# swarth100/dynfu

Measured on AMD Instinct MI355X. Metric: frames/sec (warp-solve + TSDF fuse), 512^3 vol / 2k nodes / VGA depth, higher is better.
Workload: dtype f32; 1 GPU; C2: 512^3 TSDF, 640x480 depth, 2048 nodes, k=4, 262144 vertices, 5 GN x PCG<=256 (tol 1e-6), reference-parity energy (energy.t), lambda=200; parallelism=replicas x1 (one sequence per GPU, no collective), ranks_seen=1, repeats=5

## Files before the change

### dynfu_amd/csrc/capi.cpp

```cpp
#include <hip/hip_runtime.h>

#include <cmath>
#include <cstdarg>
#include <cstdio>
#include <cstring>
#include <map>
#include <mutex>
#include <new>
#include <utility>
#include <vector>

#include "../../include/dynfu_amd.h"
#include "kernels.hpp"
#include "dev_switch.hpp"
#include "solve.hpp"
#include "solve6.hpp"

namespace {

thread_local char g_err[512] = "";

int fail(int code, const char* fmt, ...) {
    va_list ap;
    va_start(ap, fmt);
    vsnprintf(g_err, sizeof(g_err), fmt, ap);
    va_end(ap);
    return code;
}

int hip_fail(hipError_t e, const char* what) {
    return fail(e == hipErrorNoDevice ? DFA_ERR_NO_GPU : DFA_ERR_HIP, "%s: %s", what, hipGetErrorString(e));
}

#define REQUIRE(cond, msg) \
    if (!(cond)) return fail(DFA_ERR_INVALID, "%s: %s", __func__, msg)
#define HIP_TRY(expr)                                  \
    do {                                               \
        hipError_t e_ = (expr);                        \
        if (e_ != hipSuccess) return hip_fail(e_, #expr); \
    } while (0)

inline hipStream_t S(dfa_stream_t s) { return (hipStream_t)s; }

bool volume_args_ok(const void* vol, int X, int Y, int Z) { return vol && X > 0 && Y > 0 && Z > 0; }

template <class T>
T& stream_scratch(hipStream_t s) {
    static std::mutex mu;
    static std::map<std::pair<int, hipStream_t>, T> table;
    int dev = 0;
    (void)hipGetDevice(&dev);
    std::lock_guard<std::mutex> lock(mu);
    return table[std::make_pair(dev, s)];
}

struct GridScratch {
    dfa::KnnGridView v{};
    int cap_nodes = 0;
    void release() {
        (void)hipFree(v.desc), (void)hipFree(v.cell_count), (void)hipFree(v.cell_start);
        (void)hipFree(v.node_cell), (void)hipFree(v.sorted);
        v         = dfa::KnnGridView{};
        cap_nodes = 0;
    }
    hipError_t reserve(int D_needed) {
        if (D_needed <= cap_nodes) return hipSuccess;
        const int D = D_needed + D_needed / 4 + 64;
        release();
        hipError_t e;
        if ((e = hipMalloc((void**)&v.desc, sizeof(dfa::KnnGridDesc))) != hipSuccess) return e;
        if ((e = hipMalloc((void**)&v.cell_count, sizeof(int32_t) * dfa::KNN_GRID_MAX_CELLS)) != hipSuccess) return e;
        if ((e = hipMalloc((void**)&v.cell_start, sizeof(int32_t) * (dfa::KNN_GRID_MAX_CELLS + 1))) != hipSuccess)
            return e;
        if ((e = hipMalloc((void**)&v.node_cell, sizeof(int32_t) * (size_t)D)) != hipSuccess) return e;
        if ((e = hipMalloc((void**)&v.sorted, sizeof(float4) * (size_t)D)) != hipSuccess) return e;
        cap_nodes = D;
        return hipSuccess;
    }
};

struct PointGridScratch {
    dfa::PointGridView v{};
    int cap_points = 0;
    void release() {
        (void)hipFree(v.g.desc), (void)hipFree(v.g.cell_count), (void)hipFree(v.g.cell_start);
        (void)hipFree(v.g.node_cell), (void)hipFree(v.g.sorted), (void)hipFree(v.chunk_sums);
        (void)hipFree(v.bbox_partials);
        v          = dfa::PointGridView{};
        cap_points = 0;
    }
    hipError_t reserve(int n_needed) {
        if (n_needed <= cap_points) return hipSuccess;
        const int n = n_needed + n_needed / 4 + 1024;
        release();
        hipError_t e;
        const size_t cells = dfa::PGRID_MAX_CELLS;
        if ((e = hipMalloc((void**)&v.g.desc, sizeof(dfa::KnnGridDesc))) != hipSuccess) return e;
        if ((e = hipMalloc((void**)&v.g.cell_count, sizeof(int32_t) * cells)) != hipSuccess) return e;
        if ((e = hipMalloc((void**)&v.g.cell_start, sizeof(int32_t) * (cells + 1))) != hipSuccess) return e;
        if ((e = hipMalloc((void**)&v.g.node_cell, sizeof(int32_t) * (size_t)n)) != hipSuccess) return e;
        if ((e = hipMalloc((void**)&v.g.sorted, sizeof(float4) * (size_t)n)) != hipSuccess) return e;
        if ((e = hipMalloc((void**)&v.chunk_sums, sizeof(int32_t) * (cells / dfa::PGRID_CHUNK))) != hipSuccess) return e;
        if ((e = hipMalloc((void**)&v.bbox_partials, sizeof(float) * 6 * dfa::PGRID_BBOX_BLOCKS)) != hipSuccess) return e;
        cap_points = n;
        return hipSuccess;
    }
};

struct McScratch {
    int32_t* seg_off    = nullptr;
    int32_t* chunk_sums = nullptr;
    long cap_segs       = 0;
    hipError_t reserve(long nsegs) {
        if (nsegs <= cap_segs) return hipSuccess;
        (void)hipFree(seg_off), (void)hipFree(chunk_sums);
        seg_off = chunk_sums = nullptr, cap_segs = 0;
        hipError_t e;
        if ((e = hipMalloc((void**)&seg_off, sizeof(int32_t) * (size_t)(nsegs + 1))) != hipSuccess) return e;
        if ((e = hipMalloc((void**)&chunk_sums, sizeof(int32_t) * (size_t)dfa::mc_scan_chunks(nsegs))) != hipSuccess)
            return e;
        cap_segs = nsegs;
        return hipSuccess;
    }
};
struct McIndexedScratch {
    McScratch vert;
    int32_t* idx_off = nullptr;
    long cap_segs    = 0;
    hipError_t reserve(long nsegs) {
        hipError_t e = vert.reserve(nsegs);
        if (e != hipSuccess || nsegs <= cap_segs) return e;
        (void)hipFree(idx_off);
        idx_off = nullptr, cap_segs = 0;
        if ((e = hipMalloc((void**)&idx_off, sizeof(int32_t) * (size_t)(nsegs + 1))) != hipSuccess) return e;
        cap_segs = nsegs;
        return hipSuccess;
    }
};

bool want_grid(int D, long n_query) { return D >= 64 && ((long)D * n_query >= (1L << 22) || D >= 1024); }

}

struct dfa_solver {
    int max_D, max_N, k;
    size_t max_R;
    int ell_cap;
    dfa::SolveView v;
    dfa::SolveState* state;
    double* cost_partials;
    unsigned int* ticket;
    std::vector<void*> blocks;
    GridScratch grid;
    bool has_problem;
    bool timing;
    std::vector<hipEvent_t> events;
    std::vector<int> ev_pcg, ev_asm;
    size_t ev_used;
    int timed_solves = 0;
    dfa::MbGraphCache mb_graphs;
    dfa::TeamPcg team;
    bool deterministic = false;
    bool just_reset = false;
    long long* iters_total = nullptr;
    dfa_overlap_fn overlap_fn = nullptr;
    void* overlap_user        = nullptr;
    int* host_flag = nullptr;
};

struct dfa_solver6 {
    int max_D, max_N, k;
    dfa::Solve6View v;
    dfa::Solve6State* state;
    float* raw_w;
    int32_t* raw_reg;
    const float* node_dq;
    std::vector<void*> blocks;
    GridScratch grid;
    bool has_problem;
    std::map<int, hipGraphExec_t> pcg_graphs;
    int last_launches = 0;
    static constexpr int S6_RING = 4;
    int* mirror = nullptr;
    hipEvent_t done_ev[S6_RING] = {};
    int slot_gn[S6_RING] = {};
    unsigned long long solve_seq = 0, folded = 0;
    int pred[dfa::S6_HIST] = {};
    struct BudgetKey { int D, N, num_iter, gn_iter, linear_iter; float tol, tol_first, tol_decay, tol_adapt, gn_tol; } budget_key = {};
    bool graph_disabled = false;
    hipStream_t capture_stream = nullptr;
    bool timing = false;
    std::vector<hipEvent_t> events;
    size_t ev_used = 0;
    int pcg_key_D = -1;
};

namespace {
template <class T>
int plan6_alloc(dfa_solver6* s, T** out, size_t count) {
    void* p      = nullptr;
    hipError_t e = hipMalloc(&p, sizeof(T) * (count ? count : 1));
    if (e != hipSuccess) return hip_fail(e, "hipMalloc (solver6 plan)");
    s->blocks.push_back(p);
    *out = (T*)p;
    return DFA_OK;
}
}

namespace {
int timing_begin(dfa_solver* s, hipStream_t st) {
    if (s->ev_used + 2 > s->events.size()) {
        for (int i = 0; i < 2; ++i) {
            hipEvent_t e;
            if (hipEventCreate(&e) != hipSuccess) return -1;
            s->events.push_back(e);
        }
    }
    const int idx = (int)s->ev_used;
    s->ev_used += 2;
    (void)hipEventRecord(s->events[idx], st);
    return idx;
}
void timing_end(dfa_solver* s, int idx, hipStream_t st) {
    if (idx >= 0) (void)hipEventRecord(s->events[idx + 1], st);
}

template <class T>
int plan_alloc(dfa_solver* s, T** out, size_t count) {
    void* p       = nullptr;
    hipError_t e  = hipMalloc(&p, sizeof(T) * (count ? count : 1));
    if (e != hipSuccess) return hip_fail(e, "hipMalloc (solver plan)");
    s->blocks.push_back(p);
    *out = (T*)p;
    return DFA_OK;
}
}

extern "C" {

const char* dfa_last_error(void) { return g_err; }

const char* dfa_version(void) { return "dynfu_amd 0.1 (gfx950, HIP)"; }

int dfa_abi_version(void) { return DFA_ABI_VERSION; }

size_t dfa_abi_struct_size(int id) {
    switch (id) {
        case DFA_STRUCT_SOLVE_PARAMS: return sizeof(dfa_solve_params);
        case DFA_STRUCT_SOLVE_STATS: return sizeof(dfa_solve_stats);
        case DFA_STRUCT_SOLVE_TIMING: return sizeof(dfa_solve_timing);
        case DFA_STRUCT_SOLVE6_PARAMS: return sizeof(dfa_solve6_params);
        case DFA_STRUCT_SOLVE6_STATS: return sizeof(dfa_solve6_stats);
        case DFA_STRUCT_SOLVE6_TIMING: return sizeof(dfa_solve6_timing);
        default: return 0;
    }
}


int dfa_compute_dists(const uint16_t* depth, int depth_step, uint16_t* dists, int dists_step, int cols, int rows,
                      float fx, float fy, float cx, float cy, dfa_stream_t stream) {
    REQUIRE(depth && dists, "null image");
    REQUIRE(cols > 0 && rows > 0, "empty image");
    REQUIRE(depth_step >= cols * 2 && dists_step >= cols * 2, "row step smaller than a row");
    REQUIRE(fx != 0.f && fy != 0.f, "zero focal length");
    HIP_TRY(dfa::launch_compute_dists(depth, depth_step, dists, dists_step, cols, rows, fx, fy, cx, cy, S(stream)));
    return DFA_OK;
}

int dfa_tsdf_clear(uint32_t* volume, int X, int Y, int Z, dfa_stream_t stream) {
    REQUIRE(volume_args_ok(volume, X, Y, Z), "bad volume");
    HIP_TRY(dfa::launch_tsdf_clear(volume, X, Y, Z, S(stream)));
    return DFA_OK;
}

size_t dfa_tsdf_occupancy_bytes(int X, int Y, int Z) {
    return X > 0 && Y > 0 && Z > 0 ? dfa::occ_dims(X, Y, Z).bytes() : 0;
}

int dfa_tsdf_clear_occ(uint32_t* volume, int X, int Y, int Z, uint8_t* occupancy, dfa_stream_t stream) {
    REQUIRE(volume_args_ok(volume, X, Y, Z), "bad volume");
    REQUIRE(occupancy, "null occupancy map");
    HIP_TRY(dfa::launch_tsdf_clear(volume, X, Y, Z, S(stream)));
    HIP_TRY(hipMemsetAsync(occupancy, 0, dfa::occ_dims(X, Y, Z).bytes(), S(stream)));
    return DFA_OK;
}

static int integrate_common(bool fused, const uint16_t* dists, int dists_step, int cols, int rows, uint32_t* volume,
                            int X, int Y, int Z, const float voxel_size[3], float trunc_dist, int max_weight,
                            const float vol2cam[12], float fx, float fy, float cx, float cy, uint8_t* occupancy,
                            dfa_stream_t stream, bool occupancy_known = false) {
    REQUIRE(volume_args_ok(volume, X, Y, Z), "bad volume");
    REQUIRE(dists && cols > 0 && rows > 0 && dists_step >= cols * 2, "bad dists image");
    REQUIRE(voxel_size && vol2cam, "null parameter block");
    REQUIRE(trunc_dist > 0.f, "trunc_dist must be positive");
    REQUIRE(max_weight >= 0 && max_weight <= 65535, "max_weight must fit the 16-bit weight");
    HIP_TRY(dfa::launch_tsdf_integrate(fused, dists, dists_step, cols, rows, volume, X, Y, Z, voxel_size, trunc_dist,
                                       max_weight, vol2cam, fx, fy, cx, cy, occupancy, occupancy_known, S(stream)));
    return DFA_OK;
}

int dfa_tsdf_integrate_occ(const uint16_t* dists, int dists_step, int cols, int rows, uint32_t* volume, int X, int Y, int Z,
                           const float voxel_size[3], float trunc_dist, int max_weight, const float vol2cam[12], float fx,
                           float fy, float cx, float cy, uint8_t* occupancy, dfa_stream_t stream) {
    REQUIRE(occupancy, "null occupancy map");
    return integrate_common(false, dists, dists_step, cols, rows, volume, X, Y, Z, voxel_size, trunc_dist, max_weight, vol2cam,
                            fx, fy, cx, cy, occupancy, stream);
}

int dfa_tsdf_clear_integrate_occ(const uint16_t* dists, int dists_step, int cols, int rows, uint32_t* volume, int X, int Y,
                                 int Z, const float voxel_size[3], float trunc_dist, int max_weight,
                                 const float vol2cam[12], float fx, float fy, float cx, float cy, uint8_t* occupancy,
                                 dfa_stream_t stream) {
    REQUIRE(occupancy, "null occupancy map");
    return integrate_common(true, dists, dists_step, cols, rows, volume, X, Y, Z, voxel_size, trunc_dist, max_weight, vol2cam,
                            fx, fy, cx, cy, occupancy, stream);
}
// ... 507 lines not shown
        grid = &gs.v;
    }
    HIP_TRY(dfa::launch_correspond(canon_vertices, canon_normals, n_canon, live_vertices, n_live, out_vertices,
                                   out_normals, out_index, grid, S(stream)));
    return DFA_OK;
}

int dfa_correspond_projective(const float* vertices, const float* normals, int n, const float* vmap, int vmap_step,
                              const float* nmap, int nmap_step, int cols, int rows, float fx, float fy, float cx, float cy,
                              float dist_thresh, float min_cosine, float* out_vertices, float* out_normals,
                              int32_t* out_pixel, dfa_stream_t stream) {
    REQUIRE(n >= 0 && (n == 0 || vertices), "bad vertices");
    REQUIRE(vmap && cols > 0 && rows > 0 && vmap_step >= 16 * cols, "bad vertex map");
    REQUIRE(!nmap || nmap_step >= 16 * cols, "bad normal map pitch");
    REQUIRE(!out_normals || nmap, "normals requested without a normal map");
    REQUIRE(fx > 0.f && fy > 0.f && dist_thresh >= 0.f, "bad intrinsics / threshold");
    REQUIRE(((uintptr_t)vmap & 15) == 0 && (vmap_step & 15) == 0 && ((uintptr_t)nmap & 15) == 0 && (!nmap || (nmap_step & 15) == 0),
            "maps must be 16-byte aligned float4 images");
    HIP_TRY(dfa::launch_correspond_projective(vertices, normals, n, vmap, vmap_step, nmap, nmap_step, cols, rows, fx, fy, cx,
                                              cy, dist_thresh, min_cosine, out_vertices, out_normals, out_pixel,
                                              S(stream)));
    return DFA_OK;
}


int dfa_solver_create(int max_D, int max_N, int k, dfa_solver** out) {
    REQUIRE(out, "null out");
    *out = nullptr;
    REQUIRE(max_D > 0 && max_N >= 0, "bad sizes");
    REQUIRE(k >= 1 && k <= DFA_MAX_KNN, "k out of range 1..16");
    REQUIRE(max_D <= dfa::solve_pcg_max_nodes(), "more nodes than a plan supports (32768)");
    int ndev = 0;
    if (hipGetDeviceCount(&ndev) != hipSuccess || ndev == 0) return fail(DFA_ERR_NO_GPU, "no HIP device");
    dfa_solver* s = new (std::nothrow) dfa_solver();
    REQUIRE(s, "out of host memory");
    s->max_D = max_D, s->max_N = max_N, s->k = k;
    s->max_R       = (size_t)max_N + (size_t)max_D * k;
    s->ell_cap     = 256;
    s->has_problem = false;
    s->timing      = false;
    {
        const char* e    = getenv("DFA_ASSEMBLE_DETERMINISTIC");
        s->deterministic = e && atoi(e) != 0;
    }
    s->ev_used     = 0;
    std::memset(&s->v, 0, sizeof(s->v));
    const size_t R = s->max_R, D = (size_t)max_D;
    int rc = DFA_OK;
#define A(field, count) \
    if (rc == DFA_OK) rc = plan_alloc(s, &s->v.field, (count))
    A(ridx, R * k);
    A(rw, R * k);
    A(rtau, R);
    A(rb, R * 3);
    A(re, R * (size_t)dfa::solve_rec_words(k));
    A(reg_idx, D * k);
    A(blk_hist, D * (dfa::SOLVE_TG_BLOCKS + 1));
    A(node_ptr, D + 1);
    A(node_list, R * k);
    A(ell, D * s->ell_cap);
    A(ell_cnt, D);
    A(diag, D);
    A(g, D * 3);
    A(g_base, D * 3);
    A(t_base, D * 3);
    A(pk_perm, D);
    A(pk_perm2, D);
    A(pk_vals, D * s->ell_cap);
    A(pk_cols, D * s->ell_cap);
    A(mb_x, D);
    A(mb_r, D);
    A(mb_p, D);
    A(mb_s, D);
    A(mb_w, D);
    A(mb_u[0], D);
    A(mb_u[1], D);
    A(mb_m[0], D);
    A(mb_m[1], D);
    A(mb_t[0], D);
    A(mb_t[1], D);
    A(mb_gpart[0], (size_t)dfa::solve_mb_blocks(max_D));
    A(mb_gpart[1], (size_t)dfa::solve_mb_blocks(max_D));
    A(mb_dpart[0], (size_t)dfa::solve_mb_blocks(max_D));
    A(mb_dpart[1], (size_t)dfa::solve_mb_blocks(max_D));
    A(t, D * 3);
    A(huber, D);
    A(node_dq_out, D * 8);
#undef A
    if (rc == DFA_OK) {
        hipError_t e = s->grid.reserve(max_D);
        if (e != hipSuccess) rc = hip_fail(e, "hipMalloc (node grid)");
    }
    if (rc == DFA_OK && dfa::solve_team_pcg_fits(max_D) && (max_D > 2048 || dfa::kDevAB)) {
        s->v.team_stride = (max_D + 3) & ~3;
        rc = plan_alloc(s, &s->v.team_ctl, 1);
        const size_t areas = (size_t)3 * dfa::solve_team_pcg_rounds();
        if (rc == DFA_OK) rc = plan_alloc(s, &s->v.team_mt, areas * s->v.team_stride);
        if (rc == DFA_OK) rc = plan_alloc(s, &s->v.team_words, dfa::solve_team_pcg_words());
        if (rc == DFA_OK && (hipMemset(s->v.team_ctl, 0, sizeof(dfa::TeamCtl)) != hipSuccess ||
                             hipMemset(s->v.team_words, 0, sizeof(unsigned long long) * dfa::solve_team_pcg_words()) != hipSuccess ||
                             hipMemset(s->v.team_mt, 0, sizeof(float2) * areas * (size_t)s->v.team_stride) != hipSuccess))
            rc = fail(DFA_ERR_HIP, "hipMemset (team PCG)");
        if (rc == DFA_OK && hipHostMalloc((void**)&s->team.host_abort, sizeof(int), hipHostMallocDefault) == hipSuccess) {
            *s->team.host_abort = 0;
            s->team.ctl = s->v.team_ctl;
            if (const char* e0 = dfa::dev_env("DFA_MB_TEAM_EPOCH")) s->team.epoch = (unsigned)std::strtoul(e0, nullptr, 0);
        }
    }
    if (rc == DFA_OK) rc = plan_alloc(s, &s->state, 1);
    if (rc == DFA_OK) rc = plan_alloc(s, &s->iters_total, 1);
    if (rc == DFA_OK && hipMemset(s->iters_total, 0, sizeof(long long)) != hipSuccess) rc = DFA_ERR_HIP;
    if (rc == DFA_OK && hipHostMalloc((void**)&s->host_flag, 4 * sizeof(int), hipHostMallocDefault) != hipSuccess) s->host_flag = nullptr;
    if (rc == DFA_OK) rc = plan_alloc(s, &s->cost_partials, std::max<size_t>((R + 255) / 256 + 1, 1024) + 1024);
    if (rc == DFA_OK) rc = plan_alloc(s, &s->ticket, 64);
    if (rc == DFA_OK && hipMemset(s->ticket, 0, 64 * sizeof(unsigned int)) != hipSuccess)
        rc = fail(DFA_ERR_HIP, "hipMemset (ticket)");
    if (rc != DFA_OK) {
        dfa_solver_destroy(s);
        return rc;
    }
    *out = s;
    return DFA_OK;
}

void dfa_solver_destroy(dfa_solver* s) {
    if (!s) return;
    for (void* p : s->blocks) (void)hipFree(p);
    s->grid.release();
    for (hipEvent_t e : s->events) (void)hipEventDestroy(e);
    if (s->host_flag) (void)hipHostFree(s->host_flag);
    if (s->team.host_abort) (void)hipHostFree(s->team.host_abort);
    s->mb_graphs.release();
    delete s;
}

int dfa_solver_set_problem(dfa_solver* s, const float* node_pos, const float* node_dq, const float* node_w, int D,
                           const float* canon_vertices, const float* canon_normals, const float* live_vertices,
                           const float* live_normals, int N, dfa_stream_t stream) {
    (void)canon_normals;
    (void)live_normals;
    REQUIRE(s, "null plan");
    REQUIRE(node_pos && node_dq && node_w && D > 0, "no nodes");
    REQUIRE(N >= 0 && (N == 0 || (canon_vertices && live_vertices)), "bad vertex arrays");
    if (D > s->max_D || N > s->max_N)
        return fail(DFA_ERR_CAPACITY, "dfa_solver_set_problem: D=%d N=%d exceed the plan (max_D=%d max_N=%d)", D, N,
                    s->max_D, s->max_N);
    dfa::SolveView& v = s->v;
    v.N = N, v.D = D, v.k = s->k, v.Dpad = (D + 3) & ~3, v.ell_cap = s->ell_cap;
    v.deterministic = s->deterministic ? 1 : 0;
    v.node_pos = node_pos, v.node_dq = node_dq, v.node_w = node_w;
    v.canon = canon_vertices, v.live = live_vertices;
    hipStream_t st = S(stream);
    const dfa::KnnGridView* grid = nullptr;
    if (want_grid(D, (long)N + D)) {
        HIP_TRY(dfa::knn_grid_build(s->grid.v, node_pos, D, st));
        grid = &s->grid.v;
    }
    if (N > 0) HIP_TRY(dfa::launch_knn(node_pos, node_w, D, canon_vertices, N, s->k, v.ridx, v.rw, grid, st));
    HIP_TRY(dfa::launch_knn(node_pos, node_w, D, node_pos, D, s->k, v.reg_idx, nullptr, grid, st));
    HIP_TRY(dfa::solve_build_graph(v, s->state, s->ticket, 64, st));
    s->has_problem = true;
    s->just_reset  = true;
    return DFA_OK;
}

int dfa_solver_set_deterministic(dfa_solver* s, int on) {
    REQUIRE(s, "null plan");
    s->deterministic = on != 0;
    return DFA_OK;
}

int dfa_solver_solve(dfa_solver* s, const dfa_solve_params* p, dfa_stream_t stream) {
    REQUIRE(s && p, "null plan / params");
    REQUIRE(s->has_problem, "set_problem has not been called");
    REQUIRE(p->num_iter >= 0 && p->nonlinear_iter >= 0 && p->linear_iter >= 0, "negative iteration count");
    REQUIRE(p->tukey_offset > 0.f && p->psi_data > 0.f, "tukey_offset / psi_data must be positive");
    REQUIRE(p->lambda >= 0.f && std::isfinite(p->lambda), "lambda must be non-negative and finite");
    const dfa::SolveView& v = s->v;
    hipStream_t st          = S(stream);
    if (!s->just_reset) HIP_TRY(dfa::solve_reset(v, s->state, s->ticket, 64, st));
    s->just_reset = false;
    const double w_reg    = std::sqrt((double)p->lambda / ((double)v.D * (double)v.k));
    const float w_reg_f   = (float)w_reg;
    const float w_reg_sq  = w_reg_f * w_reg_f;
    if (s->timing) s->timed_solves += 1;
    if (s->host_flag) s->host_flag[0] = s->host_flag[1] = 0;
    s->mb_graphs.call = 0;
    int not_launched = 0;
    int gn_launched = 0;
    bool huber_done = false;
    const bool big_budget = (long)p->num_iter * p->nonlinear_iter > 8;
    const bool pcg_async  = dfa::solve_pcg_is_async(v, &s->team, p->linear_iter);
    const bool no_regradient = dfa::dev_env("DFA_NO_REGRADIENT") != nullptr;
    for (int outer = 0; outer < p->num_iter; ++outer) {
        if (s->host_flag && s->host_flag[1] == 2) s->host_flag[1] = 0;
        int gn_in_outer = 0;
        for (int gn = 0; gn < p->nonlinear_iter; ++gn) {
            if (big_budget && gn_in_outer >= 4 && gn_in_outer % 4 == 0 && s->host_flag && !s->host_flag[1] && pcg_async) {
                HIP_TRY(hipMemcpyAsync(&s->host_flag[1], &s->state->converged, sizeof(int), hipMemcpyDeviceToHost, st));
                HIP_TRY(hipStreamSynchronize(st));
            }
            if (s->host_flag && s->host_flag[1]) {
                ++not_launched;
                continue;
            }
            ++gn_in_outer;
            if (gn > 0 && p->gn_tol == 0.f && p->lambda > 0.f && !no_regradient) {
                int evg = s->timing ? timing_begin(s, st) : -1;
                HIP_TRY(dfa::solve_regradient(v, s->state, st));
                timing_end(s, evg, st);
                if (evg >= 0) s->ev_asm.push_back(evg);
                if (s->overlap_fn) s->overlap_fn(s->overlap_user, stream, gn_launched);
                ++gn_launched;
                int evr = s->timing ? timing_begin(s, st) : -1;
                HIP_TRY(dfa::solve_pcg(v, s->state, p->linear_iter, p->pcg_tol, s->host_flag, &s->mb_graphs, &s->team,
                                       evr >= 0 ? s->events[evr + 1] : nullptr, st));
                if (evr >= 0) s->ev_pcg.push_back(evr);
                continue;
            }
            const bool with_huber = gn == 0 && outer == p->num_iter - 1;
            HIP_TRY(dfa::solve_linearise(v, s->state, s->cost_partials, s->ticket, gn == 0, gn == 0 ? 0 : 1,
                                         p->gn_tol, p->tukey_offset, p->psi_data, w_reg_sq, with_huber ? p->psi_reg : 0.f, nullptr, st));
            huber_done |= with_huber;
            int ev = s->timing ? timing_begin(s, st) : -1;
            HIP_TRY(dfa::solve_assemble(v, s->state, gn == 0 && p->nonlinear_iter > 1, w_reg_sq, st));
            timing_end(s, ev, st);
            if (ev >= 0) s->ev_asm.push_back(ev);
            if (s->overlap_fn) s->overlap_fn(s->overlap_user, stream, gn_launched);
            ++gn_launched;
            ev = s->timing ? timing_begin(s, st) : -1;
            HIP_TRY(dfa::solve_pcg(v, s->state, p->linear_iter, p->pcg_tol, s->host_flag, &s->mb_graphs, &s->team,
                                   ev >= 0 ? s->events[ev + 1] : nullptr, st));
            if (ev >= 0) s->ev_pcg.push_back(ev);
        }
    }
    if (s->overlap_fn && gn_launched == 0) s->overlap_fn(s->overlap_user, stream, -1);
    if (not_launched) HIP_TRY(dfa::solve_count_noop(s->state, not_launched, st));
    const bool no_weights = p->num_iter == 0 || p->nonlinear_iter == 0;
    if (!huber_done) HIP_TRY(dfa::solve_huber(v, p->psi_reg, st));
    HIP_TRY(dfa::solve_linearise(v, s->state, s->cost_partials, s->ticket, no_weights ? 1 : 0, 2, 0.f,
                                 p->tukey_offset, p->psi_data, w_reg_sq, 0.f, s->timing ? s->iters_total : nullptr, st));
    return DFA_OK;
}

int dfa_solver_set_overlap_callback(dfa_solver* s, dfa_overlap_fn fn, void* user) {
    REQUIRE(s, "null plan");
    s->overlap_fn = fn, s->overlap_user = user;
    return DFA_OK;
}

const float* dfa_solver_translations(const dfa_solver* s) { return s ? s->v.t : nullptr; }
const float* dfa_solver_node_dq(const dfa_solver* s) { return s ? s->v.node_dq_out : nullptr; }
const float* dfa_solver_tukey_weights(const dfa_solver* s) { return s ? s->v.rtau : nullptr; }
const float* dfa_solver_huber_weights(const dfa_solver* s) { return s ? s->v.huber : nullptr; }
const int32_t* dfa_solver_data_graph(const dfa_solver* s) { return s ? s->v.ridx : nullptr; }
const int32_t* dfa_solver_reg_graph(const dfa_solver* s) { return s ? s->v.reg_idx : nullptr; }
const float* dfa_solver_matrix_entries(const dfa_solver* s) { return s ? (const float*)s->v.ell : nullptr; }
const int32_t* dfa_solver_matrix_row_lengths(const dfa_solver* s) { return s ? s->v.ell_cnt : nullptr; }
const float* dfa_solver_gradient(const dfa_solver* s) { return s ? s->v.g : nullptr; }

int dfa_solver_warp_to_live(dfa_solver* s, const float* normals, float* out_vertices, float* out_normals,
                            dfa_stream_t stream) {
    REQUIRE(s && s->has_problem, "no problem set");
    REQUIRE(out_vertices || s->v.N == 0, "null output");
    HIP_TRY(dfa::launch_warp_graph(s->v.node_pos, s->v.node_dq_out, s->v.node_w, s->k, s->v.ridx, s->v.canon, normals,
                                   s->v.N, out_vertices, out_normals, S(stream)));
    return DFA_OK;
}

int dfa_solver_get_stats(dfa_solver* s, dfa_solve_stats* host_out, dfa_stream_t stream) {
    REQUIRE(s && host_out, "null plan / out");
    dfa::SolveState h;
    HIP_TRY(hipMemcpyAsync(&h, s->state, sizeof(h), hipMemcpyDeviceToHost, S(stream)));
    HIP_TRY(hipStreamSynchronize(S(stream)));
    host_out->initial_cost = h.initial_cost;
    host_out->final_cost   = h.final_cost;
    host_out->gn_iters     = h.gn_iters;
    host_out->pcg_iters    = h.pcg_iters;
    host_out->max_row_nnz  = h.max_row_nnz;
    host_out->gn_noop      = h.gn_noop;
    if (dfa::dev_env("DFA_PCG_PROFILE_PRINT"))
        fprintf(stderr, "pcg phase cycles: spmv %lld  red_pAp %lld  update %lld  red_rz %lld  p_update+barrier %lld  loop %lld  (iters %d)\n",
                h.prof[0], h.prof[1], h.prof[2], h.prof[3], h.prof[4], h.prof[5], h.pcg_iters);
    if (dfa::dev_env("DFA_PCG_PROFILE_PRINT"))
        fprintf(stderr, "assemble block 7 cycles: init %lld  list+hash %lld  reduce+barrier %lld  compact %lld   (raw prof[6] %lld prof[7] %lld)\n",
                h.prof[6] / 1000000, h.prof[6] % 1000000, h.prof[7] / 1000000, h.prof[7] % 1000000, h.prof[6], h.prof[7]);
    if (h.overflow)
        return fail(DFA_ERR_CAPACITY, "normal-matrix row wider than the plan's ELL capacity (%d > %d)", h.max_row_nnz,
                    s->ell_cap);
    return DFA_OK;
}

int dfa_solver_enable_timing(dfa_solver* s, int enable) {
    REQUIRE(s, "null plan");
    s->timing = enable != 0;
    if (enable == 1) {
        s->ev_used = 0, s->timed_solves = 0;
        s->ev_pcg.clear(), s->ev_asm.clear();
        if (s->iters_total) HIP_TRY(hipMemset(s->iters_total, 0, sizeof(long long)));
    }
    return DFA_OK;
}

int dfa_solver_team_pcg_info(dfa_solver* s, int* launches, int* aborts, int* disabled) {
    REQUIRE(s, "null plan");
    if (launches) *launches = (int)std::min<long>(s->team.launches, 0x7fffffffL);
    if (aborts) *aborts = s->team.host_abort ? *(volatile int*)s->team.host_abort : 0;
    if (disabled) *disabled = (!s->team.ctl || s->team.disabled) ? 1 : 0;
    return DFA_OK;
}

int dfa_solver_get_timing(dfa_solver* s, dfa_solve_timing* out, dfa_stream_t stream) {
    REQUIRE(s && out, "null plan / out");
// ... 218 lines not shown
                if (seen == dfa::S6_MIRROR_SKIPPED) pred = pred > 1 ? pred - 1 : 1;
                else if (seen > 0) pred = std::max(seen, pred - 1);
                else if (seen < 0) pred = std::max(pred, -2 * seen);
            }
        }
        if (reset) {
            std::memset(s->pred, 0, sizeof(s->pred));
            s->folded = n;
        }
    } else {
        s->folded = n + 1 >= 2 ? n - 1 : 0;
        std::memset(s->pred, 0, sizeof(s->pred));
    }
    int* mirror_slot = s->mirror ? s->mirror + slot * dfa::S6_HIST : nullptr;
    if (mirror_slot) {
        if (n >= (unsigned long long)dfa_solver6::S6_RING) HIP_TRY(hipEventSynchronize(s->done_ev[slot]));
        std::memset(mirror_slot, 0, dfa::S6_HIST * sizeof(int));
        s->slot_gn[slot] = p.num_iter * p.gn_iter;
    }
    if (s->pcg_key_D != s->v.D) {
        for (auto& g : s->pcg_graphs) (void)hipGraphExecDestroy(g.second);
        s->pcg_graphs.clear();
        s->pcg_key_D = s->v.D;
    }
    for (int outer = 0; outer < p.num_iter; ++outer)
        for (int gn = 0; gn < p.gn_iter; ++gn) {
            auto mark = [&]() {
                if (!s->timing) return;
                if (s->ev_used == s->events.size()) {
                    hipEvent_t e;
                    if (hipEventCreate(&e) != hipSuccess) return;
                    s->events.push_back(e);
                }
                (void)hipEventRecord(s->events[s->ev_used++], st);
            };
            const int gi = outer * p.gn_iter + gn;
            mark();
            HIP_TRY(dfa::s6_linearise(s->v, s->state, img, p, gn == 0, gi, gn, 0, st));
            mark();
            HIP_TRY(dfa::s6_assemble(s->v, s->state, p, gn, st));
            mark();
            int launches = p.linear_iter;
            if (adaptive && gi < dfa::S6_HIST && s->pred[gi] > 0)
                launches = std::min(p.linear_iter, s->pred[gi] + std::max(2, s->pred[gi] / 4));
            bool replayed = false;
            if (!s->graph_disabled) {
                auto it = s->pcg_graphs.find(launches);
                if (it == s->pcg_graphs.end()) {
                    hipGraph_t g = nullptr;
                    hipGraphExec_t ge = nullptr;
                    bool ok = s->capture_stream || hipStreamCreateWithFlags(&s->capture_stream, hipStreamNonBlocking) == hipSuccess;
                    ok = ok && hipStreamBeginCapture(s->capture_stream, hipStreamCaptureModeThreadLocal) == hipSuccess;
                    if (ok) {
                        const hipError_t le = dfa::s6_pcg_n(s->v, s->state, launches, s->capture_stream);
                        const hipError_t ce = hipStreamEndCapture(s->capture_stream, &g);
                        ok = le == hipSuccess && ce == hipSuccess && g && hipGraphInstantiate(&ge, g, nullptr, nullptr, 0) == hipSuccess;
                        if (g) (void)hipGraphDestroy(g);
                    }
                    if (ok) {
                        it = s->pcg_graphs.emplace(launches, ge).first;
                    } else {
                        (void)hipGetLastError();
                        s->graph_disabled = true;
                    }
                }
                if (it != s->pcg_graphs.end()) {
                    HIP_TRY(hipGraphLaunch(it->second, st));
                    replayed = true;
                }
            }
            if (!replayed) HIP_TRY(dfa::s6_pcg_n(s->v, s->state, launches, st));
            s->last_launches += launches + 1;
            mark();
            HIP_TRY(dfa::s6_update(s->v, s->state, launches, p.linear_iter, gi < dfa::S6_HIST ? mirror_slot : nullptr, gi, 1, st));
        }
    if (early && p.num_iter * p.gn_iter > 0) {
        const int gi = p.num_iter * p.gn_iter;
        HIP_TRY(dfa::s6_linearise(s->v, s->state, img, p, 0, gi, p.gn_iter, 1, st));
        HIP_TRY(dfa::s6_update(s->v, s->state, 0, p.linear_iter, nullptr, gi, 0, st));
    }
    if (mirror_slot) HIP_TRY(hipEventRecord(s->done_ev[slot], st));
    return DFA_OK;
}

int dfa_solver6_enable_timing(dfa_solver6* s, int enable) {
    REQUIRE(s, "null plan");
    s->timing = enable != 0;
    return DFA_OK;
}

int dfa_solver6_get_timing(dfa_solver6* s, dfa_solve6_timing* out, dfa_stream_t stream) {
    REQUIRE(s && out, "null plan / out");
    HIP_TRY(hipStreamSynchronize(S(stream)));
    std::memset(out, 0, sizeof(*out));
    for (size_t i = 0; i + 3 < s->ev_used; i += 4) {
        float a = 0.f, b = 0.f, c = 0.f;
        HIP_TRY(hipEventElapsedTime(&a, s->events[i], s->events[i + 1]));
        HIP_TRY(hipEventElapsedTime(&b, s->events[i + 1], s->events[i + 2]));
        HIP_TRY(hipEventElapsedTime(&c, s->events[i + 2], s->events[i + 3]));
        out->linearise_ms += a, out->assemble_ms += b, out->pcg_ms += c;
        out->gn_iterations += 1;
    }
    if (s->has_problem && s->v.D > 0) {
        std::vector<int32_t> cnt((size_t)s->v.D);
        HIP_TRY(hipMemcpy(cnt.data(), s->v.bcnt, sizeof(int32_t) * cnt.size(), hipMemcpyDeviceToHost));
        for (int32_t c : cnt) out->matrix_blocks += c;
    }
    return DFA_OK;
}

const float* dfa_solver6_node_dq(const dfa_solver6* s) { return s ? s->v.dq : nullptr; }
static_assert(DFA_SOLVE6_ROW_BLOCKS == dfa::S6_ROW_BLOCKS, "row capacity of the C ABI and of the plan (S6_MAXSLOT of solve6.hip)");
const float* dfa_solver6_matrix_blocks(const dfa_solver6* s) { return s ? s->v.bvals : nullptr; }
const int32_t* dfa_solver6_matrix_columns(const dfa_solver6* s) { return s ? s->v.bcols : nullptr; }
const int32_t* dfa_solver6_matrix_row_blocks(const dfa_solver6* s) { return s ? s->v.bcnt : nullptr; }
const float* dfa_solver6_gradient(const dfa_solver6* s) { return s ? s->v.g : nullptr; }
const float* dfa_solver6_step(const dfa_solver6* s) { return s ? s->v.x : nullptr; }
const int32_t* dfa_solver6_data_graph(const dfa_solver6* s) { return s ? s->v.idx_nat : nullptr; }
const int32_t* dfa_solver6_reg_graph(const dfa_solver6* s) { return s ? s->v.reg_idx : nullptr; }

int dfa_solver6_warp(dfa_solver6* s, float* out_vertices, float* out_normals, dfa_stream_t stream) {
    REQUIRE(s && s->has_problem, "no problem set");
    REQUIRE(out_vertices, "null output");
    HIP_TRY(dfa::s6_warp(s->v, s->v.dq, out_vertices, out_normals, S(stream)));
    return DFA_OK;
}

int dfa_solver6_get_stats(dfa_solver6* s, dfa_solve6_stats* out, dfa_stream_t stream) {
    REQUIRE(s && out, "null argument");
    dfa::Solve6State h;
    HIP_TRY(hipMemcpyAsync(&h, s->state, sizeof(h), hipMemcpyDeviceToHost, S(stream)));
    HIP_TRY(hipStreamSynchronize(S(stream)));
    out->initial_cost = h.initial_cost, out->final_cost = h.final_cost;
    out->gn_iters = h.gn_iters, out->pcg_iters = h.pcg_iters;
    out->gn_solves = h.gn_solves, out->gn_rejected = h.gn_rejected, out->gn_converged = h.gn_converged, out->hist_n = h.hist_n;
    out->valid_first = (long long)h.valid_first, out->valid_last = (long long)h.valid_last;
    out->max_row_blocks = h.max_row_blocks, out->overflow = h.overflow;
    out->pcg_short = h.pcg_short, out->pcg_launches = s->last_launches;
    static_assert(DFA_SOLVE6_HIST == dfa::S6_HIST, "history length of the C ABI and of the state block");
    for (int i = 0; i < DFA_SOLVE6_HIST; ++i) {
        const bool in = i < h.hist_n;
        out->valid_hist[i] = in ? (long long)h.valid_hist[i] : 0ll;
        out->stop_hist[i] = in ? h.stop_hist[i] : 0;
        out->cost_hist[i] = in ? h.cost_hist[i] : 0.0;
        out->pcg_rel_hist[i] = in ? h.pcg_rel_hist[i] : 0.f;
        out->pcg_tol_hist[i] = in ? h.pcg_tol_hist[i] : 0.f;
        out->pcg_it_hist[i] = in ? h.pcg_it_hist[i] : 0;
    }
    return h.overflow ? fail(DFA_ERR_CAPACITY, "a block row of the normal matrix exceeded the plan's capacity") : DFA_OK;
}

}

#ifdef DFA_S6_DEBUG
extern "C" __attribute__((visibility("default"))) int dfa_dev_solver6_ptrs(dfa_solver6* s, void** out) {
    const dfa::Solve6View& v = s->v;
    void* p[] = {v.utab, v.pair_ptr, v.pair_list, v.bcnt, v.bfu, (void*)v.node_ptr, (void*)v.node_list, v.bcols, v.bvals, v.g,
                 (void*)v.idx, v.rec, nullptr, v.mnode, v.rslot};
    out[18] = v.minv;
    for (size_t i = 0; i < sizeof(p) / sizeof(p[0]); ++i) out[i] = p[i];
    out[15] = (void*)(size_t)v.cap, out[16] = (void*)(size_t)v.D, out[17] = (void*)(size_t)v.N;
    return 0;
}
#endif
```

### dynfu_amd/csrc/solve.hip

```cpp
#include <hip/hip_runtime.h>
#include <cstring>

#include <algorithm>
#include <map>
#include <mutex>

#include <float.h>

#include "dq_device.hpp"
#include "dev_switch.hpp"
#include "kernels.hpp"
#include "pcg_rules.hpp"
#include "solve.hpp"

namespace dfa {


constexpr int TG_BLOCKS = SOLVE_TG_BLOCKS;

__global__ __launch_bounds__(1024) void tg_count_kernel(const int32_t* __restrict__ ridx, size_t total, int D,
                                                        int32_t* __restrict__ blk_hist ) {
    extern __shared__ int32_t hist[];
    for (int i = threadIdx.x; i < D; i += blockDim.x) hist[i] = 0;
    __syncthreads();
    const size_t chunk = (total + TG_BLOCKS - 1) / TG_BLOCKS;
    const size_t beg = chunk * blockIdx.x, end = min(beg + chunk, total);
    for (size_t e = beg + threadIdx.x; e < end; e += blockDim.x) {
        const int n = ridx[e];
        if (n >= 0) atomicAdd(&hist[n], 1);
    }
    __syncthreads();
    for (int i = threadIdx.x; i < D; i += blockDim.x) blk_hist[(size_t)blockIdx.x * D + i] = hist[i];
}

__global__ __launch_bounds__(256) void tg_colscan_kernel(int32_t* __restrict__ blk_hist , int D) {
    const int i = blockIdx.x * blockDim.x + threadIdx.x;
    if (i >= D) return;
    constexpr int G = 32;
    static_assert(TG_BLOCKS % G == 0, "workgroups of the counting sort in groups");
    int run = 0;
    for (int b0 = 0; b0 < TG_BLOCKS; b0 += G) {
        int h[G];
#pragma unroll
        for (int b = 0; b < G; ++b) h[b] = blk_hist[(size_t)(b0 + b) * D + i];
#pragma unroll
        for (int b = 0; b < G; ++b) {
            blk_hist[(size_t)(b0 + b) * D + i] = run;
            run += h[b];
        }
    }
    blk_hist[(size_t)TG_BLOCKS * D + i] = run;
}

__global__ __launch_bounds__(1024) void tg_fill_kernel(const int32_t* __restrict__ ridx, size_t total, int D,
                                                       const int32_t* __restrict__ blk_base ,
                                                       int32_t* __restrict__ node_ptr, uint32_t* __restrict__ node_list) {
    extern __shared__ int32_t cursor[];
    __shared__ int32_t wave_tot[16];
    __shared__ int32_t carry_sh;
    const int lane = threadIdx.x & 63, wave = threadIdx.x >> 6;
    if (threadIdx.x == 0) carry_sh = 0;
    __syncthreads();
    for (int base = 0; base < D; base += 1024) {
        const int i = base + threadIdx.x;
        const int v = i < D ? blk_base[(size_t)TG_BLOCKS * D + i] : 0;
        const int incl = wave_inclusive_scan(v);
        if (lane == 63) wave_tot[wave] = incl;
        __syncthreads();
        int off = carry_sh + incl - v;
        for (int w = 0; w < wave; ++w) off += wave_tot[w];
        if (i < D) {
            cursor[i] = off + blk_base[(size_t)blockIdx.x * D + i];
            if (blockIdx.x == 0) node_ptr[i] = off;
        }
        __syncthreads();
        if (threadIdx.x == 1023) carry_sh = off + v;
        __syncthreads();
    }
    if (blockIdx.x == 0 && threadIdx.x == 0) node_ptr[D] = carry_sh;
    const size_t chunk = (total + TG_BLOCKS - 1) / TG_BLOCKS;
    const size_t beg = chunk * blockIdx.x, end = min(beg + chunk, total);
    for (size_t e = beg + threadIdx.x; e < end; e += blockDim.x) {
        const int n = ridx[e];
        if (n >= 0) node_list[atomicAdd(&cursor[n], 1)] = (uint32_t)e;
    }
}


template <int K>
__device__ __forceinline__ void load_row_graph(const SolveView& s, size_t r, int (&n)[K], float (&w)[K]) {
    if (s.k == K) {
#pragma unroll
        for (int q = 0; q < K / 4; ++q) {
            const int4 iv   = reinterpret_cast<const int4*>(s.ridx + r * K)[q];
            const float4 wv = reinterpret_cast<const float4*>(s.rw + r * K)[q];
            n[4 * q] = iv.x, n[4 * q + 1] = iv.y, n[4 * q + 2] = iv.z, n[4 * q + 3] = iv.w;
            w[4 * q] = wv.x, w[4 * q + 1] = wv.y, w[4 * q + 2] = wv.z, w[4 * q + 3] = wv.w;
        }
    } else {
#pragma unroll
        for (int j = 0; j < K; ++j) n[j] = j < s.k ? s.ridx[r * s.k + j] : -1, w[j] = j < s.k ? s.rw[r * s.k + j] : 0.f;
    }
}

template <int K>
__device__ __forceinline__ float tukey_weight(const SolveView& s, size_t v, float tukey_offset, float psi_data) {
    const f3 c = mk3(s.canon[3 * v], s.canon[3 * v + 1], s.canon[3 * v + 2]);
    DQ sum     = dq_identity();
    int n[K];
    float w[K];
    load_row_graph<K>(s, v, n, w);
#pragma unroll
    for (int h = 0; h < K; h += 4) {
        float tx[4], ty[4], tz[4];
        DQ q[4];
#pragma unroll
        for (int jj = 0; jj < 4; ++jj) {
            const int nn = n[h + jj] >= 0 ? n[h + jj] : 0;
            tx[jj] = s.t[3 * nn], ty[jj] = s.t[3 * nn + 1], tz[jj] = s.t[3 * nn + 2];
            q[jj]  = dq_load(s.node_dq + 8 * (size_t)nn);
        }
#pragma unroll
        for (int jj = 0; jj < 4; ++jj) {
            if (n[h + jj] >= 0) {
                const DQ cur = dq_mul(dq_from_translation(tx[jj], ty[jj], tz[jj]), q[jj]);
                sum          = dq_mul(sum, dq_scale(cur, w[h + jj]));
            }
        }
    }
    const f3 warped = dq_transform(dq_normalize(sum), c);
    const float ex = s.live[3 * v] - warped.x, ey = s.live[3 * v + 1] - warped.y, ez = s.live[3 * v + 2] - warped.z;
    const float d = sqrtf(ex * ex + ey * ey + ez * ez) / tukey_offset;
    if (d < psi_data) {
        const double q = 1.0 - ((double)d * (double)d) / ((double)psi_data * (double)psi_data);
        return (float)(q * q);
    }
    return 0.f;
}

__device__ __forceinline__ void huber_node(const SolveView& s, int i, float psi_reg) {
    const DQ dq_i = dq_mul(dq_from_translation(s.t[3 * i], s.t[3 * i + 1], s.t[3 * i + 2]),
                           dq_load(s.node_dq + 8 * (size_t)i));
    float h = 0.f;
    for (int j = 0; j < s.k; ++j) {
        const int m = s.reg_idx[(size_t)i * s.k + j];
        if (m < 0) break;
        const f3 pm   = mk3(s.node_pos[3 * m], s.node_pos[3 * m + 1], s.node_pos[3 * m + 2]);
        const DQ dq_m = dq_mul(dq_from_translation(s.t[3 * m], s.t[3 * m + 1], s.t[3 * m + 2]),
                               dq_load(s.node_dq + 8 * (size_t)m));
        const f3 pa = dq_transform(dq_i, pm), pb = dq_transform(dq_m, pm);
        const float ex = pa.x - pb.x, ey = pa.y - pb.y, ez = pa.z - pb.z;
        const float err = sqrtf(ex * ex + ey * ey + ez * ez);
        h               = fabsf(err) <= psi_reg ? 1.f : psi_reg / fabsf(err);
    }
    s.huber[i] = h;
}
__global__ __launch_bounds__(256) void huber_kernel(SolveView s, float psi_reg) {
    const int i = blockIdx.x * blockDim.x + threadIdx.x;
    if (i < s.D) huber_node(s, i, psi_reg);
}

struct LineariseArgs {
    int update_weights;
    int mode;
    float gn_tol, tukey_offset, psi_data, w_reg_sq;
    long long* iters_total;
    float huber_psi;
};

constexpr int LIN_SHARDS     = 32;
constexpr int LIN_MAX_BLOCKS = 1024;

template <int K>
__global__ __launch_bounds__(256) void linearise_kernel(SolveView s, SolveState* __restrict__ st,
                                                        double* __restrict__ cost_partials,
                                                        unsigned int* __restrict__ ticket ,
                                                        LineariseArgs a) {
    __shared__ double wsum[4];
    __shared__ int is_last;
    if (a.huber_psi > 0.f)
        for (int i = blockIdx.x * blockDim.x + threadIdx.x; i < s.D; i += gridDim.x * blockDim.x) huber_node(s, i, a.huber_psi);
    if (a.mode == 2) {
        for (int i = blockIdx.x * blockDim.x + threadIdx.x; i < s.D; i += gridDim.x * blockDim.x) {
            const DQ out = dq_mul(dq_from_translation(s.t[3 * i], s.t[3 * i + 1], s.t[3 * i + 2]),
                                  dq_load(s.node_dq + 8 * (size_t)i));
            dq_store(s.node_dq_out + 8 * (size_t)i, out);
        }
        if (blockIdx.x == 0 && threadIdx.x == 0 && a.iters_total) *a.iters_total += st->pcg_iters;
    }
    if (st->converged == 1 || (st->converged && !a.update_weights)) {
        if (a.mode != 2 || (st->have_initial && !st->cost_stale)) return;
    }
    const size_t R = (size_t)s.N + (size_t)s.D * s.k;
    double c       = 0.0;
    float amax     = 0.f;
    for (size_t r = (size_t)blockIdx.x * blockDim.x + threadIdx.x; r < R; r += (size_t)gridDim.x * blockDim.x) {
        float tau;
        if (a.update_weights) {
            tau       = r < (size_t)s.N ? tukey_weight<K>(s, r, a.tukey_offset, a.psi_data) : a.w_reg_sq;
            s.rtau[r] = tau;
        } else {
            tau = s.rtau[r];
        }
        float sx = 0.f, sy = 0.f, sz = 0.f;
        {
            int n[K];
            float w[K], tx[K], ty[K], tz[K];
            load_row_graph<K>(s, r, n, w);
#pragma unroll
            for (int j = 0; j < K; ++j) {
                const int nn = n[j] >= 0 ? n[j] : 0;
                tx[j] = s.t[3 * nn], ty[j] = s.t[3 * nn + 1], tz[j] = s.t[3 * nn + 2];
            }
            float wm = 0.f;
#pragma unroll
            for (int j = 0; j < K; ++j)
                if (n[j] >= 0) sx += w[j] * tx[j], sy += w[j] * ty[j], sz += w[j] * tz[j], wm = fmaxf(wm, fabsf(w[j]));
            amax = fmaxf(amax, tau * wm * wm);
        }
        const float ex = s.rb[3 * r] - sx, ey = s.rb[3 * r + 1] - sy, ez = s.rb[3 * r + 2] - sz;
        *(float4*)(s.re + r * (size_t)solve_rec_words(s.k) + solve_rec_tail(s.k)) = make_float4(ex, ey, ez, tau);
        c += (double)tau * ((double)ex * ex + (double)ey * ey + (double)ez * ez);
    }
    c = wave_sum_all(c);
    __shared__ float wmax[4];
#pragma unroll
    for (int o = 32; o > 0; o >>= 1) amax = fmaxf(amax, __shfl_xor(amax, o, 64));
    if ((threadIdx.x & 63) == 0) wsum[threadIdx.x >> 6] = c, wmax[threadIdx.x >> 6] = amax;
    __syncthreads();
    if (threadIdx.x == 0) {
        __hip_atomic_store(&cost_partials[blockIdx.x], (wsum[0] + wsum[1]) + (wsum[2] + wsum[3]), __ATOMIC_RELAXED,
                           __HIP_MEMORY_SCOPE_AGENT);
        if (a.update_weights)
            __hip_atomic_store(&cost_partials[LIN_MAX_BLOCKS + blockIdx.x], (double)fmaxf(fmaxf(wmax[0], wmax[1]), fmaxf(wmax[2], wmax[3])),
                               __ATOMIC_RELAXED, __HIP_MEMORY_SCOPE_AGENT);
        asm volatile("s_waitcnt vmcnt(0)" ::: "memory");
        const unsigned int shard   = blockIdx.x % LIN_SHARDS;
        const unsigned int members = (gridDim.x - shard + LIN_SHARDS - 1) / LIN_SHARDS;
        const unsigned int nshards = min((unsigned int)LIN_SHARDS, gridDim.x);
        int last                   = 0;
        if (__hip_atomic_fetch_add(&ticket[shard], 1u, __ATOMIC_RELAXED, __HIP_MEMORY_SCOPE_AGENT) == members - 1) {
            __hip_atomic_store(&ticket[shard], 0u, __ATOMIC_RELAXED, __HIP_MEMORY_SCOPE_AGENT);
            if (__hip_atomic_fetch_add(&ticket[LIN_SHARDS], 1u, __ATOMIC_RELAXED, __HIP_MEMORY_SCOPE_AGENT) ==
                nshards - 1) {
                __hip_atomic_store(&ticket[LIN_SHARDS], 0u, __ATOMIC_RELAXED, __HIP_MEMORY_SCOPE_AGENT);
                last = 1;
            }
        }
        is_last = last;
    }
    __syncthreads();
    if (!is_last) return;

    __shared__ double sm[256];
    __shared__ double smx[256];
    double acc = 0.0, mx = 0.0;
    {
        constexpr int Q = LIN_MAX_BLOCKS / 256;
        double cq[Q], mq[Q];
#pragma unroll
        for (int q = 0; q < Q; ++q) {
            const unsigned int i = min(threadIdx.x + 256u * q, gridDim.x - 1);
            cq[q] = __hip_atomic_load(&cost_partials[i], __ATOMIC_RELAXED, __HIP_MEMORY_SCOPE_AGENT);
            mq[q] = a.update_weights ? __hip_atomic_load(&cost_partials[LIN_MAX_BLOCKS + i], __ATOMIC_RELAXED, __HIP_MEMORY_SCOPE_AGENT) : 0.0;
        }
#pragma unroll
        for (int q = 0; q < Q; ++q)
            if (threadIdx.x + 256u * q < gridDim.x) acc += cq[q], mx = fmax(mx, mq[q]);
    }
    sm[threadIdx.x] = acc, smx[threadIdx.x] = mx;
    __syncthreads();
    for (int o = 128; o > 0; o >>= 1) {
        if ((int)threadIdx.x < o) sm[threadIdx.x] += sm[threadIdx.x + o], smx[threadIdx.x] = fmax(smx[threadIdx.x], smx[threadIdx.x + o]);
        __syncthreads();
    }
    if (threadIdx.x == 0) {
        const double cost = sm[0];
        if (a.update_weights) st->amax = (float)smx[0];
        if (!st->have_initial) st->initial_cost = cost, st->have_initial = 1;
        if (a.mode == 0) st->done = 0;
        if (a.mode == 1 && !st->done && a.gn_tol > 0.f && (st->cost - cost) <= (double)a.gn_tol * st->cost)
            st->done = 1;
        st->cost       = cost;
        st->final_cost = cost;
        st->cost_stale = 0;
        if (a.mode != 2) st->weights_fresh = a.update_weights;
        if (a.mode != 2 && a.update_weights && st->converged == 2) st->converged = 0;
    }
}

__global__ __launch_bounds__(256) void reset_kernel(float* __restrict__ t, int n3, SolveState* __restrict__ st,
                                                    unsigned int* __restrict__ ticket, int nticket) {
    const int i = blockIdx.x * blockDim.x + threadIdx.x;
    if (i < n3) t[i] = 0.f;
    if (blockIdx.x == 0) {
        unsigned int* w = (unsigned int*)st;
        for (int j = threadIdx.x; j < (int)(sizeof(SolveState) / 4); j += blockDim.x) w[j] = 0u;
        for (int j = threadIdx.x; j < nticket; j += blockDim.x) ticket[j] = 0u;
    }
}

template <int K>
__global__ __launch_bounds__(256) void prepare_rows_kernel(SolveView s, SolveState* __restrict__ st,
                                                           unsigned int* __restrict__ ticket, int nticket) {
    const size_t R = (size_t)s.N + (size_t)s.D * s.k;
    const size_t r = (size_t)blockIdx.x * blockDim.x + threadIdx.x;
    if (r < (size_t)3 * s.D) s.t[r] = 0.f;
    if (blockIdx.x == 0) {
        unsigned int* w = (unsigned int*)st;
        for (int j = threadIdx.x; j < (int)(sizeof(SolveState) / 4); j += blockDim.x) w[j] = 0u;
        for (int j = threadIdx.x; j < nticket; j += blockDim.x) ticket[j] = 0u;
    }
    if (r >= R) return;
    const int k = s.k;
    int ids[K];
    float ws[K];
    const bool wide = k == K && K % 4 == 0;
    if (r < (size_t)s.N) {
#pragma unroll
        for (int c = 0; c < 3; ++c) s.rb[3 * r + c] = s.live[3 * r + c] - s.canon[3 * r + c];
        if (wide) load_row_graph<K>(s, r, ids, ws);
        else {
#pragma unroll
            for (int j = 0; j < K; ++j)
                if (j < k) ids[j] = s.ridx[r * k + j], ws[j] = s.rw[r * k + j];
        }
    } else {
        const int e = (int)(r - (size_t)s.N), n = e / k, m = s.reg_idx[e];
#pragma unroll
        for (int j = 0; j < K; ++j) ids[j] = -1, ws[j] = 0.f;
        if (m >= 0 && m != n) ids[0] = m, ws[0] = -1.f, ids[1] = n, ws[1] = +1.f;
        if (wide) {
#pragma unroll
            for (int q = 0; q < K / 4; ++q) {
                reinterpret_cast<int4*>(s.ridx + r * K)[q]  = make_int4(ids[4 * q], ids[4 * q + 1], ids[4 * q + 2], ids[4 * q + 3]);
                reinterpret_cast<float4*>(s.rw + r * K)[q] = make_float4(ws[4 * q], ws[4 * q + 1], ws[4 * q + 2], ws[4 * q + 3]);
            }
        } else {
#pragma unroll
            for (int j = 0; j < K; ++j)
                if (j < k) s.ridx[r * k + j] = ids[j], s.rw[r * k + j] = ws[j];
        }
        s.rb[3 * r + 0] = s.rb[3 * r + 1] = s.rb[3 * r + 2] = 0.f;
    }
    float* rec = s.re + r * (size_t)solve_rec_words(k);
    if (wide) {
        float4* rec4 = reinterpret_cast<float4*>(rec);
        if (solve_rec_ids16(k)) {
            uint32_t pk[K / 2];
#pragma unroll
            for (int j = 0; j < K / 2; ++j) {
                const uint32_t lo = ids[2 * j] < 0 ? 0xffffu : (uint32_t)ids[2 * j], hi = ids[2 * j + 1] < 0 ? 0xffffu : (uint32_t)ids[2 * j + 1];
                pk[j]             = (lo & 0xffffu) | (hi << 16);
            }
#pragma unroll
            for (int q = 0; q < K / 8; ++q)
                rec4[q] = make_float4(__uint_as_float(pk[4 * q]), __uint_as_float(pk[4 * q + 1]), __uint_as_float(pk[4 * q + 2]), __uint_as_float(pk[4 * q + 3]));
#pragma unroll
            for (int q = 0; q < K / 4; ++q) rec4[K / 8 + q] = make_float4(ws[4 * q], ws[4 * q + 1], ws[4 * q + 2], ws[4 * q + 3]);
        } else {
#pragma unroll
            for (int q = 0; q < K / 4; ++q)
                rec4[q] = make_float4(__int_as_float(ids[4 * q]), __int_as_float(ids[4 * q + 1]), __int_as_float(ids[4 * q + 2]), __int_as_float(ids[4 * q + 3]));
#pragma unroll
            for (int q = 0; q < K / 4; ++q) rec4[K / 4 + q] = make_float4(ws[4 * q], ws[4 * q + 1], ws[4 * q + 2], ws[4 * q + 3]);
        }
        return;
    }
    if (solve_rec_ids16(k)) {
        uint16_t* h = reinterpret_cast<uint16_t*>(rec);
#pragma unroll
        for (int j = 0; j < K; ++j)
            if (j < k) h[j] = ids[j] < 0 ? (uint16_t)0xffffu : (uint16_t)ids[j], rec[k / 2 + j] = ws[j];
        return;
    }
#pragma unroll
    for (int j = 0; j < K; ++j)
        if (j < k) rec[j] = __int_as_float(ids[j]), rec[k + j] = ws[j];
}


constexpr int HASH      = 512;
constexpr int HASH_MASK = HASH - 1;

struct FixedScale {
    float up;
    double down;
};
__device__ __forceinline__ FixedScale solve_fixed_scale(float amax) {
    int e = 0;
    (void)frexpf(fmaxf(amax, 1e-30f), &e);
    e = e < -80 ? -80 : e > 100 ? 100 : e;
    FixedScale f;
    f.up   = ldexpf(1.f, 40 - e);
    f.down = ldexp(1.0, e - 40);
    return f;
}
__device__ __forceinline__ FixedScale fixed_scale_for_rows(FixedScale f, int rows) {
    const int extra = 32 - __clz((unsigned)max(rows, 1) >> 22);
    if (extra > 0) f.up = ldexpf(f.up, -extra), f.down = ldexp(f.down, extra);
    return f;
}
__device__ __forceinline__ void fixed_add(long long* cell, float v, float up) {
    const float x  = truncf(fabsf(v) * up);
    const float hf = floorf(x * 2.3283064365386963e-10f);
    const uint32_t hi = (uint32_t)hf, lo = (uint32_t)fmaf(hf, -4294967296.f, x);
    atomicAdd(reinterpret_cast<unsigned long long*>(v < 0.f ? cell + HASH : cell), ((unsigned long long)hi << 32) | lo);
}

template <int K>
__device__ __forceinline__ float4 load_record(const SolveView& s, size_t r, int (&idx)[K], float (&w)[K]) {
    const float* rec = s.re + r * (size_t)solve_rec_words(s.k);
    if (s.k == K && (K % 8) == 0) {
        const float4* v = (const float4*)rec;
#pragma unroll
        for (int q = 0; q < K / 8; ++q) {
            const float4 i4 = v[q];
            const uint32_t u[4] = {__float_as_uint(i4.x), __float_as_uint(i4.y), __float_as_uint(i4.z), __float_as_uint(i4.w)};
#pragma unroll
            for (int h = 0; h < 4; ++h) {
                const int lo = (int)(u[h] & 0xffffu), hi = (int)(u[h] >> 16);
                idx[8 * q + 2 * h]     = lo == 0xffff ? -1 : lo;
                idx[8 * q + 2 * h + 1] = hi == 0xffff ? -1 : hi;
            }
        }
#pragma unroll
        for (int q = 0; q < K / 4; ++q) {
            const float4 w4 = v[K / 8 + q];
            w[4 * q] = w4.x, w[4 * q + 1] = w4.y, w[4 * q + 2] = w4.z, w[4 * q + 3] = w4.w;
        }
        return v[K / 8 + K / 4];
    }
    if (solve_rec_ids16(s.k)) {
        const uint16_t* ids = reinterpret_cast<const uint16_t*>(rec);
#pragma unroll
        for (int j = 0; j < K; ++j) {
            idx[j] = j < s.k ? (ids[j] == 0xffffu ? -1 : (int)ids[j]) : -1;
            w[j]   = j < s.k ? rec[s.k / 2 + j] : 0.f;
        }
        const float* tl = rec + solve_rec_tail(s.k);
        return make_float4(tl[0], tl[1], tl[2], tl[3]);
    }
    if (s.k == K && (K % 4) == 0) {
        const float4* v = (const float4*)rec;
#pragma unroll
        for (int q = 0; q < K / 4; ++q) {
            const float4 i4 = v[q], w4 = v[K / 4 + q];
            idx[4 * q] = __float_as_int(i4.x), idx[4 * q + 1] = __float_as_int(i4.y);
            idx[4 * q + 2] = __float_as_int(i4.z), idx[4 * q + 3] = __float_as_int(i4.w);
            w[4 * q] = w4.x, w[4 * q + 1] = w4.y, w[4 * q + 2] = w4.z, w[4 * q + 3] = w4.w;
        }
        return v[K / 2];
    }
#pragma unroll
    for (int j = 0; j < K; ++j) {
        idx[j] = j < s.k ? __float_as_int(rec[j]) : -1;
        w[j]   = j < s.k ? rec[s.k + j] : 0.f;
    }
    return make_float4(rec[2 * s.k], rec[2 * s.k + 1], rec[2 * s.k + 2], rec[2 * s.k + 3]);
}

#ifdef DFA_PCG_PROFILE
__device__ unsigned long long asm_tbuf[32768 * 8];
extern "C" __attribute__((visibility("default"))) int dfa_dev_asm_timing(unsigned long long* out, int n) {
    return (int)hipMemcpyFromSymbol(out, HIP_SYMBOL(asm_tbuf), sizeof(unsigned long long) * 8 * (size_t)n);
}
#endif

template <int K>
__global__ __launch_bounds__(256) void assemble_kernel(SolveView s, SolveState* __restrict__ st, int save_base, float amax_unset) {
    __shared__ int key[HASH];
    __shared__ long long val[2 * HASH];
    __shared__ float gpart[4][3];
    __shared__ int wave_cnt[4];
    __shared__ int ovf;
    if (st->done || st->converged) return;
    const int a = blockIdx.x;
    const int wave = threadIdx.x >> 6, lane = threadIdx.x & 63;
#ifdef DFA_PCG_PROFILE
    long long t0_ = clock64(), t1_, t2_, t3_, t4_;
    const unsigned long long w0_ = wall_clock64();
#endif
    for (int i = threadIdx.x; i < HASH; i += 256) key[i] = -1, val[i] = val[i + HASH] = 0ll;
    if (threadIdx.x == 0) ovf = 0;
    __syncthreads();
#ifdef DFA_PCG_PROFILE
    t1_ = clock64();
#endif

    const int beg = s.node_ptr[a], end = s.node_ptr[a + 1];
    const FixedScale fx = fixed_scale_for_rows(solve_fixed_scale(st->amax > 0.f ? st->amax : amax_unset), end - beg);
    float gx = 0.f, gy = 0.f, gz = 0.f, dsum = 0.f;
    for (int p = beg + (int)threadIdx.x; p < end; p += 256) {
        const uint32_t e = s.node_list[p];
        const size_t r   = e / (uint32_t)s.k;
        const int slot   = (int)(e - (uint32_t)r * (uint32_t)s.k);
        int idx[K];
        float w[K];
        const float4 et = load_record<K>(s, r, idx, w);
        float wa = 0.f;
#pragma unroll
        for (int j = 0; j < K; ++j) wa = (j == slot) ? w[j] : wa;
        const float tw = et.w * wa;
        gx += tw * et.x, gy += tw * et.y, gz += tw * et.z;
        if (et.w != 0.f) {
            uint32_t h0[K];
            int k0[K];
#pragma unroll
            for (int j = 0; j < K; ++j) {
                h0[j] = ((uint32_t)idx[j] * 2654435761u) >> (32 - 9);
                k0[j] = key[h0[j]];
            }
#pragma unroll
            for (int j = 0; j < K; ++j) {
                const int b = idx[j];
                if (b < 0) continue;
                const float v = tw * w[j];
                if (b == a) {
                    dsum += v;
                    continue;
                }
                if (k0[j] == b) {
                    fixed_add(&val[h0[j]], v, fx.up);
                    continue;
                }
                uint32_t h = h0[j];
                int cur    = k0[j];
#pragma unroll 1
                for (int probes = 0;; ++probes) {
                    if (cur == -1) cur = atomicCAS(&key[h], -1, b), cur = cur == -1 ? b : cur;
                    if (cur == b) {
// ... 682 lines not shown
                    slots4(q0, aB[j]);
                } else {
                    if (q0 + 2 >= E - nB[j]) slots2(q0 + 2, aB[j]);
                    break;
                }
            }
        }
    };
    auto publish = [&](const float (&vA)[P][NC], const float (&vB)[P][NC]) __attribute__((always_inline)) {
#pragma unroll
        for (int j = 0; j < P; ++j) {
            if (NC == 3) {
                if (rowA[j] >= 0) p_s[rowA[j]] = make_float4(vA[j][0], vA[j][NC / 2], vA[j][NC - 1], 0.f);
                if (rowB[j] >= 0) p_s[rowB[j]] = make_float4(vB[j][0], vB[j][NC / 2], vB[j][NC - 1], 0.f);
            } else {
                if (rowA[j] >= 0) p_s1[rowA[j]] = vA[j][0];
                if (rowB[j] >= 0) p_s1[rowB[j]] = vB[j][0];
            }
        }
    };
    if (NC == 3) {
        while (it < max_iter) {
            if (!(rz > 0.f)) break;
            PROF_MARK(5);
            float aA[P][NC], aB[P][NC];
            float pap_loc = 0.f;
            matvec(aA, aB);
#pragma unroll
            for (int j = 0; j < P; ++j)
#pragma unroll
                for (int c = 0; c < NC; ++c) pap_loc = fmaf(pA[j][c], aA[j][c], fmaf(pB[j][c], aB[j][c], pap_loc));
            PROF_MARK(0);
            const float pAp = block_sum_f<NT / 64>(pap_loc, red0);
            PROF_MARK(1);
            if (!(pAp > 0.f)) break;
            const float alpha = rz / pAp;
            float rzn_loc     = 0.f;
#pragma unroll
            for (int j = 0; j < P; ++j)
#pragma unroll
                for (int c = 0; c < NC; ++c) {
                    xA[j][c]  = fmaf(alpha, pA[j][c], xA[j][c]);
                    xB[j][c]  = fmaf(alpha, pB[j][c], xB[j][c]);
                    rA_[j][c] = fmaf(-alpha, aA[j][c], rA_[j][c]);
                    rB_[j][c] = fmaf(-alpha, aB[j][c], rB_[j][c]);
                    rzn_loc = fmaf(rA_[j][c], minvA[j] * rA_[j][c], fmaf(rB_[j][c], minvB[j] * rB_[j][c], rzn_loc));
                }
            PROF_MARK(2);
            const float rz_new = block_sum_f<NT / 64>(rzn_loc, red1);
            PROF_MARK(3);
            ++it;
            if (rz_new <= target) break;
            const float beta = rz_new / rz;
#pragma unroll
            for (int j = 0; j < P; ++j)
#pragma unroll
                for (int c = 0; c < NC; ++c) {
                    pA[j][c] = fmaf(beta, pA[j][c], minvA[j] * rA_[j][c]);
                    pB[j][c] = fmaf(beta, pB[j][c], minvB[j] * rB_[j][c]);
                }
            publish(pA, pB);
            rz = rz_new;
            __syncthreads();
            PROF_MARK(4);
        }
    }
    if (NC == 1) {
        float sA[P][NC], sB[P][NC], uA[P][NC], uB[P][NC];
#pragma unroll
        for (int j = 0; j < P; ++j)
#pragma unroll
            for (int c = 0; c < NC; ++c) {
                uA[j][c] = pA[j][c], uB[j][c] = pB[j][c];
                pA[j][c] = pB[j][c] = sA[j][c] = sB[j][c] = 0.f;
            }
        float gamma_old = 1.f, alpha_old = 1.f;
        __syncthreads();
        while (it < max_iter) {
            PROF_MARK(5);
            float wA[P][NC], wB[P][NC];
            matvec(wA, wB);
            float g_loc = 0.f, d_loc = 0.f;
#pragma unroll
            for (int j = 0; j < P; ++j)
#pragma unroll
                for (int c = 0; c < NC; ++c) {
                    g_loc = fmaf(rA_[j][c], uA[j][c], fmaf(rB_[j][c], uB[j][c], g_loc));
                    d_loc = fmaf(wA[j][c], uA[j][c], fmaf(wB[j][c], uB[j][c], d_loc));
                }
            PROF_MARK(0);
            const float gw = wave_total(g_loc), dw = wave_total(d_loc);
            if ((tid & 63) == 0) red0[tid >> 6] = gw, red1[tid >> 6] = dw;
            __syncthreads();
            float gamma = 0.f, delta = 0.f;
#pragma unroll
            for (int i = 0; i < NT / 64; ++i) gamma += red0[i], delta += red1[i];
            PROF_MARK(1);
            if (!(gamma > target)) break;
            const float beta  = cg_beta(it == 0, gamma, gamma_old);
            const float denom = cg_denom(it == 0, gamma, delta, beta, alpha_old);
            if (!(denom > 0.f)) break;
            const float alpha = gamma / denom;
#pragma unroll
            for (int j = 0; j < P; ++j)
#pragma unroll
                for (int c = 0; c < NC; ++c) {
                    cg_update_row(alpha, beta, uA[j][c], wA[j][c], pA[j][c], sA[j][c], xA[j][c], rA_[j][c]);
                    cg_update_row(alpha, beta, uB[j][c], wB[j][c], pB[j][c], sB[j][c], xB[j][c], rB_[j][c]);
                    uA[j][c]  = minvA[j] * rA_[j][c];
                    uB[j][c]  = minvB[j] * rB_[j][c];
                }
            ++it;
            gamma_old = gamma, alpha_old = alpha;
            PROF_MARK(2);
            publish(uA, uB);
            __syncthreads();
            PROF_MARK(4);
        }
    }
#ifdef DFA_PCG_PROFILE
    if (tid == 0 && c0 == 0)
        for (int i = 0; i < 6; ++i) st->prof[i] += pc_[i];
#endif
#pragma unroll
    for (int j = 0; j < P; ++j)
#pragma unroll
        for (int c = 0; c < NC; ++c) {
            if (rowA[j] >= 0) s.t[3 * rowA[j] + c0 + c] += xA[j][c];
            if (rowB[j] >= 0) s.t[3 * rowB[j] + c0 + c] += xB[j][c];
        }
    if (tid == 0) {
        if (NC == 3) pcg_book_launch(st, rz0, it, false);
        else pcg_book_launch_of_three(st, rz0, it, false);
    }
}


#define KDISPATCH(kernel, k, ...)                      \
    do {                                               \
        if ((k) <= 4) kernel<4> __VA_ARGS__;           \
        else if ((k) <= 8) kernel<8> __VA_ARGS__;      \
        else kernel<16> __VA_ARGS__;                   \
    } while (0)

hipError_t solve_transpose_graph(const int32_t* ridx, size_t total, int D, int32_t* blk_hist, int32_t* node_ptr,
                                 uint32_t* node_list, hipStream_t st) {
    const size_t lds = sizeof(int32_t) * (size_t)D;
    tg_count_kernel<<<TG_BLOCKS, 1024, lds, st>>>(ridx, total, D, blk_hist);
    tg_colscan_kernel<<<(D + 255) / 256, 256, 0, st>>>(blk_hist, D);
    tg_fill_kernel<<<TG_BLOCKS, 1024, lds, st>>>(ridx, total, D, blk_hist, node_ptr, node_list);
    return hipGetLastError();
}

hipError_t solve_build_graph(const SolveView& s, SolveState* state, unsigned int* ticket, int nticket, hipStream_t st) {
    const int D = s.D, N = s.N, k = s.k;
    const size_t R = (size_t)N + (size_t)D * k, total = R * k;
    const size_t threads = R > (size_t)3 * D ? R : (size_t)3 * D;
    KDISPATCH(prepare_rows_kernel, k, <<<(unsigned)((threads + 255) / 256), 256, 0, st>>>(s, state, ticket, nticket));
    const size_t lds = sizeof(int32_t) * (size_t)D;
    tg_count_kernel<<<TG_BLOCKS, 1024, lds, st>>>(s.ridx, total, D, s.blk_hist);
    tg_colscan_kernel<<<(D + 255) / 256, 256, 0, st>>>(s.blk_hist, D);
    tg_fill_kernel<<<TG_BLOCKS, 1024, lds, st>>>(s.ridx, total, D, s.blk_hist, s.node_ptr, s.node_list);
    if (s.deterministic) sort_node_lists_kernel<<<D, 256, 0, st>>>(s.node_ptr, s.node_list);
    return hipGetLastError();
}

int solve_residual_blocks(const SolveView& s) {
    const size_t R  = (size_t)s.N + (size_t)s.D * s.k;
    const size_t nb = (R + 255) / 256;
    return (int)(nb < (size_t)LIN_MAX_BLOCKS ? nb : (size_t)LIN_MAX_BLOCKS);
}

hipError_t solve_linearise(const SolveView& s, SolveState* state, double* cost_partials, unsigned int* ticket,
                           int update_weights, int mode, float gn_tol, float tukey_offset, float psi_data,
                           float w_reg_sq, float huber_psi, long long* iters_total, hipStream_t st) {
    const int nb = solve_residual_blocks(s);
    LineariseArgs a{update_weights, mode, gn_tol, tukey_offset, psi_data, w_reg_sq, iters_total, huber_psi};
    KDISPATCH(linearise_kernel, s.k, <<<nb, 256, 0, st>>>(s, state, cost_partials, ticket, a));
    return hipGetLastError();
}

hipError_t solve_reset(const SolveView& s, SolveState* state, unsigned int* ticket, int nticket, hipStream_t st) {
    reset_kernel<<<(3 * s.D + 255) / 256, 256, 0, st>>>(s.t, 3 * s.D, state, ticket, nticket);
    return hipGetLastError();
}

hipError_t solve_huber(const SolveView& s, float psi_reg, hipStream_t st) {
    huber_kernel<<<(s.D + 255) / 256, 256, 0, st>>>(s, psi_reg);
    return hipGetLastError();
}

hipError_t solve_assemble(const SolveView& s, SolveState* state, int save_base, float w_reg_sq, hipStream_t st) {
    const float amax_unset = std::max(1.0f, w_reg_sq);
    if (s.deterministic) KDISPATCH(assemble_det_kernel, s.k, <<<s.D, 256, 0, st>>>(s, state, save_base, amax_unset));
    else KDISPATCH(assemble_kernel, s.k, <<<s.D, 256, 0, st>>>(s, state, save_base, amax_unset));
    return hipGetLastError();
}

__global__ __launch_bounds__(256) void regradient_kernel(SolveView s, SolveState* __restrict__ st) {
    if (st->done || st->converged) return;
    const int a = blockIdx.x * blockDim.x + threadIdx.x;
    if (a == 0) st->cost_stale = 1, st->weights_fresh = 0;
    if (a >= s.D) return;
    const int cnt = s.ell_cnt[a];
    float sx = 0.f, sy = 0.f, sz = 0.f;
    for (int q = 0; q < cnt; ++q) {
        const float2 e = s.ell[(size_t)q * s.D + a];
        const int col  = __float_as_int(e.y);
        sx = fmaf(e.x, s.t[3 * col] - s.t_base[3 * col], sx);
        sy = fmaf(e.x, s.t[3 * col + 1] - s.t_base[3 * col + 1], sy);
        sz = fmaf(e.x, s.t[3 * col + 2] - s.t_base[3 * col + 2], sz);
    }
    s.g[3 * a] = s.g_base[3 * a] - sx, s.g[3 * a + 1] = s.g_base[3 * a + 1] - sy, s.g[3 * a + 2] = s.g_base[3 * a + 2] - sz;
}

hipError_t solve_regradient(const SolveView& s, SolveState* state, hipStream_t st) {
    regradient_kernel<<<(s.D + 255) / 256, 256, 0, st>>>(s, state);
    return hipGetLastError();
}

constexpr int MB_LPR = 16;

__device__ __forceinline__ float sum_partials_mb(const float* __restrict__ part, int n) {
    float acc = 0.f;
    for (int i = threadIdx.x & 63; i < n; i += 64) acc += part[i];
    return wave_sum_all(acc);
}

__global__ __launch_bounds__(256) void pcg_mb_init_kernel(SolveView s, SolveState* __restrict__ st) {
    __shared__ float sh[4];
    const int a = blockIdx.x * blockDim.x + threadIdx.x;
    if (a == 0) {
        st->mb_done = st->done || st->converged ? 1 : 0, st->mb_skip = st->done ? 1 : 0, st->mb_iters = 0, st->mb_rz0 = 0.f;
        if (st->converged) st->gn_noop += 1;
    }
    float rz = 0.f;
    if (a < s.D) {
        const float minv = jacobi_inv(s.diag[a]);
        const float4 r   = make_float4(s.g[3 * a], s.g[3 * a + 1], s.g[3 * a + 2], 0.f);
        const float4 z   = make_float4(minv * r.x, minv * r.y, minv * r.z, 0.f);
        const float4 zero = make_float4(0.f, 0.f, 0.f, 0.f);
        s.mb_r[a] = r, s.mb_u[0][a] = z, s.mb_x[a] = zero;
        s.mb_p[a] = s.mb_s[a] = s.mb_t[0][a] = s.mb_t[1][a] = zero;
        rz = fmaf(r.z, z.z, fmaf(r.y, z.y, r.x * z.x));
    }
    rz = wave_sum_all(rz);
    if ((threadIdx.x & 63) == 0) sh[threadIdx.x >> 6] = rz;
    __syncthreads();
    if (threadIdx.x == 0) s.mb_gpart[0][blockIdx.x] = (sh[0] + sh[1]) + (sh[2] + sh[3]);
}

__device__ __forceinline__ float group16_sum(float v) {
#pragma unroll
    for (int o = 8; o > 0; o >>= 1) v += __shfl_xor(v, o, 64);
    return v;
}

__global__ __launch_bounds__(256) void pcg_mb_step_kernel(SolveView s, SolveState* __restrict__ st, int it, float pcg_tol) {
    __shared__ float sh[2][4];
    const int nb  = solve_mb_blocks(s.D);
    const int cur = it >= 0 ? (it & 1) : 0, nxt = cur ^ 1;
    const float4* ucur  = s.mb_u[cur];
    const float4* mcur  = s.mb_m[cur];
    const float4* tprev = s.mb_t[nxt];
    const int lane16  = threadIdx.x & (MB_LPR - 1);
    const int a       = (blockIdx.x * 256 + threadIdx.x) / MB_LPR;
    const bool row_ok = a < s.D;
    const int cnt     = row_ok ? s.ell_cnt[a] : 0;
    const float2 e0   = row_ok ? s.ell[(size_t)lane16 * s.D + a] : make_float2(0.f, 0.f);
    const float2 e1   = row_ok ? s.ell[(size_t)(lane16 + MB_LPR) * s.D + a] : make_float2(0.f, 0.f);
    if (st->mb_done) return;
    const bool has0 = lane16 < cnt, has1 = lane16 + MB_LPR < cnt;
    const int col0  = has0 ? __float_as_int(e0.y) : 0, col1 = has1 ? __float_as_int(e1.y) : 0;
    const float4 uu0 = ucur[col0], uu1 = ucur[col1];
    float4 mm0 = make_float4(0.f, 0.f, 0.f, 0.f), tt0 = mm0, mm1 = mm0, tt1 = mm0;
    if (it >= 0) mm0 = mcur[col0], tt0 = tprev[col0], mm1 = mcur[col1], tt1 = tprev[col1];
    float alpha = 0.f, beta = 0.f;
    if (it >= 0) {
        float g = 0.f, d = 0.f;
        for (int i = threadIdx.x; i < nb; i += 256) g += s.mb_gpart[it & 1][i], d += s.mb_dpart[it & 1][i];
        g = wave_sum_all(g), d = wave_sum_all(d);
        if ((threadIdx.x & 63) == 0) sh[0][threadIdx.x >> 6] = g, sh[1][threadIdx.x >> 6] = d;
        __syncthreads();
        const float gamma = (sh[0][0] + sh[0][1]) + (sh[0][2] + sh[0][3]), delta = (sh[1][0] + sh[1][1]) + (sh[1][2] + sh[1][3]);
        float denom = delta;
        bool stop   = !(gamma > 0.f);
        if (it == 0) {
            const bool at_floor = pcg_at_floor(st, gamma, (double)1e-12f);
            stop                = stop || at_floor;
            if (blockIdx.x == 0 && threadIdx.x == 0) {
                st->mb_rz0 = gamma;
                if (at_floor) solve_mark_at_floor(st);
            }
        } else {
            beta  = cg_beta(false, gamma, st->mb_gamma_prev[(it + 1) & 1]);
            denom = cg_denom(false, gamma, delta, beta, st->mb_alpha_prev[(it + 1) & 1]);
            stop  = stop || gamma <= pcg_joint_target(st, pcg_tol, st->mb_rz0);
        }
        stop = stop || !(denom > 0.f);
        if (stop) {
            if (blockIdx.x == 0 && threadIdx.x == 0) st->mb_done = 1;
            return;
        }
        alpha = gamma / denom;
        if (blockIdx.x == 0 && threadIdx.x == 0) {
            st->mb_gamma_prev[it & 1] = gamma, st->mb_alpha_prev[it & 1] = alpha;
            st->mb_iters += 1;
        }
    }
    float au[3] = {0.f, 0.f, 0.f}, am[3] = {0.f, 0.f, 0.f}, at[3] = {0.f, 0.f, 0.f};
    for (int q = lane16; q < cnt; q += MB_LPR) {
        const bool first = q == lane16, second = q == lane16 + MB_LPR;
        const float2 e   = first ? e0 : second ? e1 : s.ell[(size_t)q * s.D + a];
        const int col    = __float_as_int(e.y);
        const float val  = e.x;
        const float4 uu  = first ? uu0 : second ? uu1 : ucur[col];
        au[0] = fmaf(val, uu.x, au[0]), au[1] = fmaf(val, uu.y, au[1]), au[2] = fmaf(val, uu.z, au[2]);
// ... 657 lines not shown
```

### dynfu_amd/csrc/solve.hpp

```cpp
#pragma once
#include <hip/hip_runtime.h>
#include <stdint.h>

namespace dfa {

struct SolveState {
    double initial_cost;
    double cost;
    double final_cost;
    double grad_first;
    int have_initial;
    int done;
    int gn_iters;
    int pcg_iters;
    int max_row_nnz;
    int overflow;
    int pcg_fallback;
    int split_iters;
    unsigned int split_ticket;
    int mb_done;
    int converged;
    int mb_skip, mb_iters;
    int weights_fresh;
    int gn_noop;
    int cost_stale;
    float mb_rz0, mb_gamma_prev[2], mb_alpha_prev[2];
    float amax;
    long long prof[8];
};

__host__ __device__ inline bool solve_rec_ids16(int k) { return k % 8 == 0; }
__host__ __device__ inline int solve_rec_words(int k) { return solve_rec_ids16(k) ? k + k / 2 + 4 : 2 * k + 4; }
__host__ __device__ inline int solve_rec_tail(int k) { return solve_rec_words(k) - 4; }

__device__ __forceinline__ void solve_mark_at_floor(SolveState* st) {
    if (st->weights_fresh) st->converged = 1;
    else if (!st->converged) st->converged = 2;
}

struct TeamCtl {
    unsigned int count[3];
    unsigned int abort[3];
    unsigned int finished[3];
    int iters[3];
    float rz0[3];
    unsigned int at_floor[3];
};

struct SolveView {
    int N, D, k, Dpad, ell_cap;
    int deterministic;
    const float* node_pos;
    const float* node_dq;
    const float* node_w;
    const float* canon;
    const float* live;
    int32_t* ridx;
    float* rw;
    float* rtau;
    float* rb;
    float* re;
    int32_t* reg_idx;
    int32_t* blk_hist;
    int32_t* node_ptr;
    uint32_t* node_list;
    float2* ell;
    int32_t* ell_cnt;
    float* diag;
    float* g;
    float* g_base;
    float* t_base;
    int32_t* pk_perm;
    int32_t* pk_perm2;
    float* pk_vals;
    uint16_t* pk_cols;
    float4 *mb_x, *mb_r, *mb_p, *mb_s, *mb_w, *mb_u[2], *mb_m[2], *mb_t[2];
    float *mb_gpart[2], *mb_dpart[2];
    TeamCtl* team_ctl;
    float2* team_mt;
    unsigned long long* team_words;
    int team_stride;
    float* t;
    float* huber;
    float* node_dq_out;
};

constexpr int SOLVE_TG_BLOCKS = 256;
hipError_t solve_build_graph(const SolveView& s, SolveState* state, unsigned int* ticket, int nticket, hipStream_t st);
hipError_t solve_transpose_graph(const int32_t* ridx, size_t total, int D, int32_t* blk_hist, int32_t* node_ptr,
                                 uint32_t* node_list, hipStream_t st);
int solve_residual_blocks(const SolveView& s);
hipError_t solve_linearise(const SolveView& s, SolveState* state, double* cost_partials, unsigned int* ticket,
                           int update_weights, int mode, float gn_tol, float tukey_offset, float psi_data,
                           float w_reg_sq, float huber_psi ,
                           long long* iters_total , hipStream_t st);
hipError_t solve_huber(const SolveView& s, float psi_reg, hipStream_t st);
hipError_t solve_reset(const SolveView& s, SolveState* state, unsigned int* ticket, int nticket, hipStream_t st);
hipError_t solve_assemble(const SolveView& s, SolveState* state, int save_base , float w_reg_sq,
                          hipStream_t st);
hipError_t solve_regradient(const SolveView& s, SolveState* state, hipStream_t st);
int solve_pcg_max_nodes();
__host__ __device__ inline int solve_mb_rows_per_block() { return 16; }
__host__ __device__ inline int solve_mb_blocks(int D) { return (D + 15) / 16; }
struct MbGraphCache {
    struct Entry {
        int it0 = 0, it1 = 0;
        float tol = 0.f;
        SolveView view;
        const SolveState* state = nullptr;
        hipGraphExec_t exec = nullptr;
    };
    Entry e[24];
    int used = 0;
    int pred[64] = {};
    int call     = 0;
    hipStream_t capture = nullptr;
    bool disabled = false;
    void release();
};

struct TeamPcg {
    TeamCtl* ctl    = nullptr;
    int* host_abort = nullptr;
    unsigned epoch  = 1;
    long launches   = 0;
    bool disabled   = false;
};
bool solve_team_pcg_fits(int D);
int solve_team_pcg_rounds();
size_t solve_team_pcg_words();

bool solve_pcg_is_async(const SolveView& s, const TeamPcg* team, int max_iter);
hipError_t solve_pcg(const SolveView& s, SolveState* state, int max_iter, float pcg_tol, int* host_flag ,
                     MbGraphCache* graphs , TeamPcg* team , hipEvent_t main_done,
                     hipStream_t st);
hipError_t solve_count_noop(SolveState* state, int n, hipStream_t st);

}
```

### dynfu_amd/csrc/warp.hip

```cpp
#include <hip/hip_runtime.h>

#include "dq_device.hpp"
#include "dev_switch.hpp"
#include "kernels.hpp"

namespace dfa {

constexpr int KNN_TILE = 1024;

template <int K>
struct KnnList {
    unsigned long long key[K];
    static constexpr unsigned long long EMPTY = 0x7f8000007fffffffull;
    __device__ __forceinline__ static unsigned long long pack(float dist, int idx) {
        return ((unsigned long long)__float_as_uint(dist) << 32) | (unsigned int)idx;
    }
    __device__ __forceinline__ void init() {
#pragma unroll
        for (int j = 0; j < K; ++j) key[j] = EMPTY;
    }
    __device__ __forceinline__ void push(float dist, int idx) {
        const unsigned long long x = pack(dist, idx);
        if (x < key[K - 1]) {
            key[K - 1] = x;
#pragma unroll
            for (int j = K - 1; j > 0; --j) {
                const unsigned long long a = key[j - 1], b = key[j];
                key[j - 1] = a < b ? a : b, key[j] = a < b ? b : a;
            }
        }
    }
    __device__ __forceinline__ float dist(int j) const { return __uint_as_float((unsigned int)(key[j] >> 32)); }
    __device__ __forceinline__ int raw_index(int j) const { return (int)(unsigned int)key[j]; }
    __device__ __forceinline__ int index(int j) const { return raw_index(j) == 0x7fffffff ? -1 : raw_index(j); }
    __device__ __forceinline__ void set_index(int j, int n) { key[j] = pack(__builtin_inff(), n < 0 ? 0x7fffffff : n); }
};

__device__ __forceinline__ float dist2(f3 q, float gx, float gy, float gz) {
    const float d0 = q.x - gx, d1 = q.y - gy, d2 = q.z - gz;
    return (d0 * d0 + d1 * d1) + d2 * d2;
}

template <int K>
__device__ __forceinline__ void knn_scan(const float* __restrict__ node_pos, int D, f3 q, KnnList<K>& best,
                                         float4* tile) {
    best.init();
    for (int base = 0; base < D; base += KNN_TILE) {
        const int n = min(KNN_TILE, D - base);
        __syncthreads();
        for (int j = threadIdx.x; j < n; j += blockDim.x) {
            const float* p = node_pos + 3 * (size_t)(base + j);
            tile[j]        = make_float4(p[0], p[1], p[2], 0.f);
        }
        __syncthreads();
        for (int j = 0; j < n; ++j) {
            const float4 g = tile[j];
            best.push(dist2(q, g.x, g.y, g.z), base + j);
        }
    }
}

__global__ __launch_bounds__(1024) void grid_setup_kernel(const float* __restrict__ node_pos, int D,
                                                          KnnGridDesc* __restrict__ desc,
                                                          int32_t* __restrict__ cell_count) {
    __shared__ float smin[3][16], smax[3][16];
    float mn[3] = {__builtin_inff(), __builtin_inff(), __builtin_inff()};
    float mx[3] = {-__builtin_inff(), -__builtin_inff(), -__builtin_inff()};
    for (int i = threadIdx.x; i < D; i += blockDim.x)
        for (int c = 0; c < 3; ++c) {
            const float v = node_pos[3 * (size_t)i + c];
            mn[c] = fminf(mn[c], v), mx[c] = fmaxf(mx[c], v);
        }
    for (int c = 0; c < 3; ++c) {
        for (int o = 32; o > 0; o >>= 1) {
            mn[c] = fminf(mn[c], __shfl_xor(mn[c], o, 64));
            mx[c] = fmaxf(mx[c], __shfl_xor(mx[c], o, 64));
        }
        if ((threadIdx.x & 63) == 0) smin[c][threadIdx.x >> 6] = mn[c], smax[c][threadIdx.x >> 6] = mx[c];
    }
    __syncthreads();
    for (int i = threadIdx.x; i < KNN_GRID_MAX_CELLS; i += blockDim.x) cell_count[i] = 0;
    if (threadIdx.x == 0) {
        float ext[3];
        for (int c = 0; c < 3; ++c) {
            float a = smin[c][0], b = smax[c][0];
            for (int w = 1; w < (int)(blockDim.x >> 6); ++w) a = fminf(a, smin[c][w]), b = fmaxf(b, smax[c][w]);
            desc->bmin[c] = a;
            ext[c]        = fmaxf(b - a, 0.f);
        }
        const float emax = fmaxf(ext[0], fmaxf(ext[1], ext[2]));
        float cs = cbrtf((ext[0] * ext[1] * ext[2]) / (float)D);
        cs       = fmaxf(cs, emax / (float)KNN_GRID_MAX_DIM);
        if (!(cs > 0.f)) cs = 1.f;
        desc->cs     = cs;
        desc->inv_cs = 1.f / cs;
        for (int c = 0; c < 3; ++c) {
            int n = (int)(ext[c] * desc->inv_cs) + 1;
            desc->dim[c] = min(max(n, 1), KNN_GRID_MAX_DIM);
        }
    }
}

__device__ __forceinline__ void cell_of(const KnnGridDesc& g, f3 p, int& cx, int& cy, int& cz) {
    cx = min(max((int)floorf((p.x - g.bmin[0]) * g.inv_cs), 0), g.dim[0] - 1);
    cy = min(max((int)floorf((p.y - g.bmin[1]) * g.inv_cs), 0), g.dim[1] - 1);
    cz = min(max((int)floorf((p.z - g.bmin[2]) * g.inv_cs), 0), g.dim[2] - 1);
}

__global__ __launch_bounds__(256) void grid_count_kernel(const float* __restrict__ node_pos, int D,
                                                         const KnnGridDesc* __restrict__ desc,
                                                         int32_t* __restrict__ cell_count,
                                                         int32_t* __restrict__ node_cell) {
    const int i = blockIdx.x * blockDim.x + threadIdx.x;
    if (i >= D) return;
    const KnnGridDesc g = *desc;
    int cx, cy, cz;
    cell_of(g, mk3(node_pos[3 * (size_t)i], node_pos[3 * (size_t)i + 1], node_pos[3 * (size_t)i + 2]), cx, cy, cz);
    const int c  = cx + g.dim[0] * (cy + g.dim[1] * cz);
    node_cell[i] = c;
    atomicAdd(&cell_count[c], 1);
}

__global__ __launch_bounds__(1024) void grid_scan_kernel(int32_t* __restrict__ cell_count ,
                                                         int32_t* __restrict__ cell_start) {
    __shared__ int32_t wave_tot[16];
    constexpr int PER = KNN_GRID_MAX_CELLS / 1024;
    const int base    = threadIdx.x * PER;
    int loc[PER], sum = 0;
#pragma unroll
    for (int j = 0; j < PER; ++j) loc[j] = cell_count[base + j], sum += loc[j];
    int incl        = sum;
    const int lane  = threadIdx.x & 63, wave = threadIdx.x >> 6;
#pragma unroll
    for (int o = 1; o < 64; o <<= 1) {
        const int t = __shfl_up(incl, o, 64);
        if (lane >= o) incl += t;
    }
    if (lane == 63) wave_tot[wave] = incl;
    __syncthreads();
    int off = incl - sum;
    for (int w = 0; w < wave; ++w) off += wave_tot[w];
#pragma unroll
    for (int j = 0; j < PER; ++j) {
        cell_start[base + j] = off;
        cell_count[base + j] = off;
        off += loc[j];
    }
    if (threadIdx.x == 1023) cell_start[KNN_GRID_MAX_CELLS] = off;
}

__global__ __launch_bounds__(256) void grid_fill_kernel(const float* __restrict__ node_pos, int D,
                                                        const int32_t* __restrict__ node_cell,
                                                        int32_t* __restrict__ cursor,
                                                        float4* __restrict__ sorted) {
    const int i = blockIdx.x * blockDim.x + threadIdx.x;
    if (i >= D) return;
    const int slot = atomicAdd(&cursor[node_cell[i]], 1);
    sorted[slot]   = make_float4(node_pos[3 * (size_t)i], node_pos[3 * (size_t)i + 1], node_pos[3 * (size_t)i + 2],
                                 __int_as_float(i));
}

constexpr int GRID_ONE_MAX = 8192;
__global__ __launch_bounds__(1024) void grid_build_one_kernel(const float* __restrict__ node_pos, int D,
                                                              KnnGridDesc* __restrict__ desc,
                                                              int32_t* __restrict__ cell_start,
                                                              float4* __restrict__ sorted) {
    extern __shared__ int32_t cnt[];
    __shared__ float smin[3][16], smax[3][16];
    __shared__ int32_t wave_tot[16];
    __shared__ KnnGridDesc gsh;
    const int tid = threadIdx.x, lane = tid & 63, wave = tid >> 6;
    float mn[3] = {__builtin_inff(), __builtin_inff(), __builtin_inff()};
    float mx[3] = {-__builtin_inff(), -__builtin_inff(), -__builtin_inff()};
    for (int i = tid; i < D; i += 1024)
        for (int c = 0; c < 3; ++c) {
            const float v = node_pos[3 * (size_t)i + c];
            mn[c] = fminf(mn[c], v), mx[c] = fmaxf(mx[c], v);
        }
    for (int c = 0; c < 3; ++c) {
        for (int o = 32; o > 0; o >>= 1) {
            mn[c] = fminf(mn[c], __shfl_xor(mn[c], o, 64));
            mx[c] = fmaxf(mx[c], __shfl_xor(mx[c], o, 64));
        }
        if (lane == 0) smin[c][wave] = mn[c], smax[c][wave] = mx[c];
    }
    __syncthreads();
    if (tid == 0) {
        float ext[3];
        for (int c = 0; c < 3; ++c) {
            float a = smin[c][0], b = smax[c][0];
            for (int w = 1; w < 16; ++w) a = fminf(a, smin[c][w]), b = fmaxf(b, smax[c][w]);
            gsh.bmin[c] = a;
            ext[c]      = fmaxf(b - a, 0.f);
        }
        const float emax = fmaxf(ext[0], fmaxf(ext[1], ext[2]));
        float cs = cbrtf((ext[0] * ext[1] * ext[2]) / (float)D);
        cs       = fmaxf(cs, emax / (float)KNN_GRID_MAX_DIM);
        if (!(cs > 0.f)) cs = 1.f;
        gsh.cs     = cs;
        gsh.inv_cs = 1.f / cs;
        for (int c = 0; c < 3; ++c) {
            const int n = (int)(ext[c] * gsh.inv_cs) + 1;
            gsh.dim[c]  = min(max(n, 1), KNN_GRID_MAX_DIM);
        }
        *desc = gsh;
    }
    __syncthreads();
    const KnnGridDesc g = gsh;
    const int ncells = g.dim[0] * g.dim[1] * g.dim[2];
    const int PER    = ((ncells + 16 * 64 - 1) / (16 * 64)) * 64;
    for (int j = 0; j < PER; j += 64) cnt[wave * PER + j + lane] = 0;
    __syncthreads();
    for (int i = tid; i < D; i += 1024) {
        int cx, cy, cz;
        cell_of(g, mk3(node_pos[3 * (size_t)i], node_pos[3 * (size_t)i + 1], node_pos[3 * (size_t)i + 2]), cx, cy, cz);
        atomicAdd(&cnt[cx + g.dim[0] * (cy + g.dim[1] * cz)], 1);
    }
    __syncthreads();
    int carry = 0;
    for (int j = 0; j < PER; j += 64) {
        const int idx  = wave * PER + j + lane;
        const int v    = cnt[idx];
        const int incl = wave_inclusive_scan(v);
        cnt[idx]       = carry + incl - v;
        carry += __builtin_amdgcn_readlane(incl, 63);
    }
    if (lane == 0) wave_tot[wave] = carry;
    __syncthreads();
    int off = 0;
    for (int w = 0; w < wave; ++w) off += wave_tot[w];
    for (int j = 0; j < PER; j += 64) {
        const int idx   = wave * PER + j + lane;
        const int start = cnt[idx] + off;
        cnt[idx]        = start;
        if (idx <= ncells) cell_start[idx] = start;
    }
    if (tid == 1023 && 16 * PER <= ncells) cell_start[ncells] = off + carry;
    __syncthreads();
    for (int i = tid; i < D; i += 1024) {
        const float px = node_pos[3 * (size_t)i], py = node_pos[3 * (size_t)i + 1], pz = node_pos[3 * (size_t)i + 2];
        int cx, cy, cz;
        cell_of(g, mk3(px, py, pz), cx, cy, cz);
        const int slot = atomicAdd(&cnt[cx + g.dim[0] * (cy + g.dim[1] * cz)], 1);
        sorted[slot]   = make_float4(px, py, pz, __int_as_float(i));
    }
}

__global__ __launch_bounds__(256) void pgrid_bbox_kernel(const float* __restrict__ pts, int n,
                                                         float* __restrict__ partials ) {
    __shared__ float sh[6][4];
    float mn[3] = {__builtin_inff(), __builtin_inff(), __builtin_inff()};
    float mx[3] = {-__builtin_inff(), -__builtin_inff(), -__builtin_inff()};
    for (int i = blockIdx.x * blockDim.x + threadIdx.x; i < n; i += gridDim.x * blockDim.x)
        for (int c = 0; c < 3; ++c) {
            const float v = pts[3 * (size_t)i + c];
            mn[c] = fminf(mn[c], v), mx[c] = fmaxf(mx[c], v);
        }
    for (int c = 0; c < 3; ++c) {
        for (int o = 32; o > 0; o >>= 1) {
            mn[c] = fminf(mn[c], __shfl_xor(mn[c], o, 64));
            mx[c] = fmaxf(mx[c], __shfl_xor(mx[c], o, 64));
        }
        if ((threadIdx.x & 63) == 0) sh[c][threadIdx.x >> 6] = mn[c], sh[3 + c][threadIdx.x >> 6] = mx[c];
    }
    __syncthreads();
    if (threadIdx.x < 6) {
        const int c = threadIdx.x;
        float a     = sh[c][0];
        for (int w = 1; w < 4; ++w) a = c < 3 ? fminf(a, sh[c][w]) : fmaxf(a, sh[c][w]);
        partials[6 * blockIdx.x + c] = a;
    }
}

__global__ __launch_bounds__(64) void pgrid_finalize_kernel(const float* __restrict__ partials, int nblocks, int n,
                                                            KnnGridDesc* __restrict__ desc) {
    float mn[3] = {__builtin_inff(), __builtin_inff(), __builtin_inff()};
    float mx[3] = {-__builtin_inff(), -__builtin_inff(), -__builtin_inff()};
    for (int b = threadIdx.x; b < nblocks; b += 64)
        for (int c = 0; c < 3; ++c) mn[c] = fminf(mn[c], partials[6 * b + c]), mx[c] = fmaxf(mx[c], partials[6 * b + 3 + c]);
    for (int c = 0; c < 3; ++c)
        for (int o = 32; o > 0; o >>= 1) {
            mn[c] = fminf(mn[c], __shfl_xor(mn[c], o, 64));
            mx[c] = fmaxf(mx[c], __shfl_xor(mx[c], o, 64));
        }
    if (threadIdx.x == 0) {
        float ext[3];
        for (int c = 0; c < 3; ++c) desc->bmin[c] = mn[c], ext[c] = fmaxf(mx[c] - mn[c], 0.f);
        const float emax = fmaxf(ext[0], fmaxf(ext[1], ext[2]));
        const bool large = n > 500000;
        float cs = (large ? 0.5f : 0.7f) * cbrtf((ext[0] * ext[1] * ext[2]) / (float)n);
        cs       = fmaxf(cs, emax / (float)(large ? PGRID_MAX_DIM : 128));
        if (!(cs > 0.f)) cs = 1.f;
        desc->cs = cs, desc->inv_cs = 1.f / cs;
        const int cap = large ? PGRID_MAX_DIM : 128;
        for (int c = 0; c < 3; ++c) desc->dim[c] = min(max((int)(ext[c] * desc->inv_cs) + 1, 1), cap);
    }
}

__device__ __forceinline__ int pgrid_cells(const KnnGridDesc& g) { return g.dim[0] * g.dim[1] * g.dim[2]; }

__global__ __launch_bounds__(256) void pgrid_clear_kernel(const KnnGridDesc* __restrict__ desc,
                                                          int32_t* __restrict__ cell_count) {
    const int nc = pgrid_cells(*desc);
    for (int i = blockIdx.x * blockDim.x + threadIdx.x; i < nc; i += gridDim.x * blockDim.x) cell_count[i] = 0;
}

__global__ __launch_bounds__(256) void pgrid_sum_kernel(const KnnGridDesc* __restrict__ desc,
                                                        const int32_t* __restrict__ cell_count,
                                                        int32_t* __restrict__ chunk_sums) {
    __shared__ int sh[4];
    const int nc = pgrid_cells(*desc), base = blockIdx.x * PGRID_CHUNK;
    int sum = 0;
    for (int i = base + threadIdx.x; i < min(base + PGRID_CHUNK, nc); i += 256) sum += cell_count[i];
    for (int o = 32; o > 0; o >>= 1) sum += __shfl_xor(sum, o, 64);
    if ((threadIdx.x & 63) == 0) sh[threadIdx.x >> 6] = sum;
    __syncthreads();
    if (threadIdx.x == 0) chunk_sums[blockIdx.x] = sh[0] + sh[1] + sh[2] + sh[3];
}

__global__ __launch_bounds__(256) void pgrid_chunkscan_kernel(int32_t* __restrict__ chunk_sums, int chunks) {
    __shared__ int wsum[4];
    constexpr int PER = (PGRID_MAX_CELLS / PGRID_CHUNK + 255) / 256;
    int loc[PER], sum = 0;
#pragma unroll
    for (int j = 0; j < PER; ++j) {
        const int i = (int)threadIdx.x * PER + j;
        loc[j]      = i < chunks ? chunk_sums[i] : 0;
        sum += loc[j];
    }
    int incl       = sum;
    const int lane = threadIdx.x & 63, wave = threadIdx.x >> 6;
#pragma unroll
    for (int o = 1; o < 64; o <<= 1) {
        const int t = __shfl_up(incl, o, 64);
        if (lane >= o) incl += t;
    }
    if (lane == 63) wsum[wave] = incl;
    __syncthreads();
    int off = incl - sum;
    for (int w = 0; w < wave; ++w) off += wsum[w];
#pragma unroll
    for (int j = 0; j < PER; ++j) {
        const int i = (int)threadIdx.x * PER + j;
        if (i < chunks) chunk_sums[i] = off;
        off += loc[j];
    }
}

__global__ __launch_bounds__(256) void pgrid_scan_kernel(const KnnGridDesc* __restrict__ desc,
                                                         int32_t* __restrict__ cell_count ,
                                                         int32_t* __restrict__ cell_start,
                                                         const int32_t* __restrict__ chunk_sums) {
    __shared__ int sh[4], sh2[4];
    const int nc = pgrid_cells(*desc), base = blockIdx.x * PGRID_CHUNK;
    if (base >= nc) return;
    if (threadIdx.x < 4) sh[threadIdx.x] = threadIdx.x == 0 ? chunk_sums[blockIdx.x] : 0;
    constexpr int PER = PGRID_CHUNK / 256;
    const int first   = base + threadIdx.x * PER;
    static_assert(PER % 4 == 0, "cells per thread in groups of four");
    const bool whole = first + PER <= nc;
    int loc[PER], sum = 0;
    if (whole) {
#pragma unroll
        for (int q = 0; q < PER / 4; ++q) {
            const int4 c4 = reinterpret_cast<const int4*>(cell_count + first)[q];
            loc[4 * q] = c4.x, loc[4 * q + 1] = c4.y, loc[4 * q + 2] = c4.z, loc[4 * q + 3] = c4.w;
        }
#pragma unroll
        for (int j = 0; j < PER; ++j) sum += loc[j];
    } else {
#pragma unroll
        for (int j = 0; j < PER; ++j) loc[j] = first + j < nc ? cell_count[first + j] : 0, sum += loc[j];
    }
    int incl       = sum;
    const int lane = threadIdx.x & 63, wave = threadIdx.x >> 6;
#pragma unroll
    for (int o = 1; o < 64; o <<= 1) {
        const int t = __shfl_up(incl, o, 64);
        if (lane >= o) incl += t;
    }
    if (lane == 63) sh2[wave] = incl;
    __syncthreads();
    int off = sh[0] + sh[1] + sh[2] + sh[3] + incl - sum;
    for (int w = 0; w < wave; ++w) off += sh2[w];
    if (whole) {
        int st[PER];
#pragma unroll
        for (int j = 0; j < PER; ++j) st[j] = off, off += loc[j];
#pragma unroll
        for (int q = 0; q < PER / 4; ++q) {
            const int4 v = make_int4(st[4 * q], st[4 * q + 1], st[4 * q + 2], st[4 * q + 3]);
            reinterpret_cast<int4*>(cell_start + first)[q] = v;
            reinterpret_cast<int4*>(cell_count + first)[q] = v;
        }
        if (first + PER == nc) cell_start[nc] = off;
        return;
    }
#pragma unroll
    for (int j = 0; j < PER; ++j) {
        if (first + j < nc) {
            cell_start[first + j] = off;
            cell_count[first + j] = off;
            off += loc[j];
            if (first + j == nc - 1) cell_start[nc] = off;
        }
    }
}

template <int K, bool TIGHT = false>
__device__ __forceinline__ void knn_grid_query(const KnnGridDesc& g, const int32_t* __restrict__ cell_start,
                                               const float4* __restrict__ sorted, f3 q, KnnList<K>& best, bool rescan = false) {
    static_assert(!TIGHT || K == 1, "the tight stop bound re-scans the own cell: 1-NN only");
    best.init();
    int cx, cy, cz;
    cell_of(g, q, cx, cy, cz);
    float margin = 0.f;
    float wall[3][2] = {{0.f, 0.f}, {0.f, 0.f}, {0.f, 0.f}};
    bool inside      = false;
    if (TIGHT) {
        const float ux = (q.x - g.bmin[0]) * g.inv_cs - (float)cx, uy = (q.y - g.bmin[1]) * g.inv_cs - (float)cy,
                    uz = (q.z - g.bmin[2]) * g.inv_cs - (float)cz;
        const float m = fminf(fminf(fminf(ux, 1.f - ux), fminf(uy, 1.f - uy)), fminf(uz, 1.f - uz));
        margin        = m > 0.f ? m : 0.f;
        inside        = m >= 0.f;
        const float u[3] = {ux, uy, uz};
#pragma unroll
        for (int c = 0; c < 3; ++c) wall[c][0] = fmaxf(u[c] - 1e-3f, 0.f) * g.cs, wall[c][1] = fmaxf(1.f - u[c] - 1e-3f, 0.f) * g.cs;
    }
    const int rmax = max(g.dim[0], max(g.dim[1], g.dim[2]));
    int r_first    = 0;
    auto scan_range = [&](int beg, int end) __attribute__((always_inline)) {
        constexpr int KNN_BATCH = 4;
        for (int j = beg; j < end; j += KNN_BATCH) {
            float4 n[KNN_BATCH];
#pragma unroll
            for (int t = 0; t < KNN_BATCH; ++t) n[t] = sorted[min(j + t, end - 1)];
#pragma unroll
            for (int t = 0; t < KNN_BATCH; ++t)
                if (j + t < end) best.push(dist2(q, n[t].x, n[t].y, n[t].z), __float_as_int(n[t].w));
        }
    };
    auto scan_block3 = [&]() __attribute__((always_inline)) {
        const int x0 = max(cx - 1, 0), x1 = min(cx + 1, g.dim[0] - 1);
        int rbeg[9], rend[9];
#pragma unroll
        for (int i = 0; i < 9; ++i) {
            const int z = cz - 1 + i / 3, y = cy - 1 + i % 3;
            const bool in = z >= 0 && z < g.dim[2] && y >= 0 && y < g.dim[1];
            const int c   = in ? g.dim[0] * (y + g.dim[1] * z) : 0;
            const int b = cell_start[c + x0], e = cell_start[c + x1 + 1];
            rbeg[i] = in ? b : 0, rend[i] = in ? e : 0;
        }
        constexpr int order[9] = {4, 1, 3, 5, 7, 0, 2, 6, 8};
#pragma unroll
        for (int i = 0; i < 9; ++i) scan_range(rbeg[order[i]], rend[order[i]]);
    };
    if (TIGHT) {
        const int c0 = cx + g.dim[0] * (cy + g.dim[1] * cz);
        scan_range(cell_start[c0], cell_start[c0 + 1]);
        const float b0 = fmaxf(margin - 1e-3f, 0.f) * g.cs;
        if (best.dist(K - 1) < b0 * b0 * 0.9999f) return;
        {
            const float d0 = best.dist(K - 1);
            int rbeg[9], rend[9];
#pragma unroll
            for (int i = 0; i < 9; ++i) {
                const int dz = i / 3 - 1, dy = i % 3 - 1, z = cz + dz, y = cy + dy;
                const float ey = dy < 0 ? wall[1][0] : dy > 0 ? wall[1][1] : 0.f, ez = dz < 0 ? wall[2][0] : dz > 0 ? wall[2][1] : 0.f;
                const float rb2 = ey * ey + ez * ez;
                const bool keep = !inside || !(d0 < rb2 * 0.9999f);
                const bool xl   = keep && (!inside || !(d0 < (rb2 + wall[0][0] * wall[0][0]) * 0.9999f));
                const bool xr   = keep && (!inside || !(d0 < (rb2 + wall[0][1] * wall[0][1]) * 0.9999f));
                const bool own  = dy == 0 && dz == 0;
                const bool mid  = keep && (!own || (xl && xr));
                const bool in   = z >= 0 && z < g.dim[2] && y >= 0 && y < g.dim[1] && (xl || xr || mid);
                const int x0 = max(xl ? cx - 1 : (mid ? cx : cx + 1), 0), x1 = min(xr ? cx + 1 : (mid ? cx : cx - 1), g.dim[0] - 1);
                const int c  = in ? g.dim[0] * (y + g.dim[1] * z) : 0;
                const bool some = in && x0 <= x1;
                const int b = cell_start[c + (some ? x0 : 0)], e = cell_start[c + (some ? x1 + 1 : 0)];
                rbeg[i] = some ? b : 0, rend[i] = some ? e : 0;
            }
#pragma unroll
            for (int i = 0; i < 9; ++i) scan_range(rbeg[i], rend[i]);
        }
        const float b1 = fmaxf(1.f + margin - 1e-3f, 0.f) * g.cs;
        if (best.dist(K - 1) < b1 * b1 * 0.9999f) return;
        r_first = 2;
        constexpr int RB = 4;
        auto reach = [&](float r, float w) { return r > w ? (int)fminf((r - w) * g.inv_cs, 1e6f) + 1 : 0; };
        float rad   = best.dist(K - 1) < 3.0e38f ? sqrtf(best.dist(K - 1)) * 1.0001f : 2.f * g.cs;
        bool settled = false;
        for (int attempt = 0; attempt < RB; ++attempt) {
            const float rad_p = attempt > 0 && !rescan ? rad - g.cs : -1.f;
            const int nzl = reach(rad, wall[2][0]), nzh = reach(rad, wall[2][1]), nyl = reach(rad, wall[1][0]), nyh = reach(rad, wall[1][1]);
            const bool ball = inside && !settled && max(max(nzl, nzh), max(nyl, nyh)) <= RB &&
                              max(reach(rad, wall[0][0]), reach(rad, wall[0][1])) <= RB;
            if (__ballot(ball) == 0ull) break;
            int zl = 0, zh = 0;
#pragma unroll
            for (int v = 1; v <= RB; ++v) {
                if (__ballot(ball && nzl >= v) != 0ull) zl = v;
                if (__ballot(ball && nzh >= v) != 0ull) zh = v;
            }
            for (int sz = 0; sz <= 2 * max(zl, zh); ++sz) {
                const int dz = (sz & 1) ? (sz + 1) / 2 : -(sz / 2);
                if (dz > zh || -dz > zl) continue;
                const float ez = dz == 0 ? 0.f : (dz < 0 ? wall[2][0] : wall[2][1]) + (float)(abs(dz) - 1) * g.cs;
                int rb[2 * RB + 1], re[2 * RB + 1], pb[2 * RB + 1], pe[2 * RB + 1];
#pragma unroll
                for (int i = 0; i <= 2 * RB; ++i) {
                    const int dy   = i - RB;
                    const float ey = dy == 0 ? 0.f : (dy < 0 ? wall[1][0] : wall[1][1]) + (float)(abs(dy) - 1) * g.cs;
                    const float rem = rad * rad - ey * ey - ez * ez;
                    const int z = cz + dz, y = cy + dy;
                    const bool row = ball && rem >= 0.f && dz <= nzh && -dz <= nzl && dy <= nyh && -dy <= nyl && z >= 0 &&
                                     z < g.dim[2] && y >= 0 && y < g.dim[1];
                    const float sx = sqrtf(fmaxf(rem, 0.f));
                    const int x0 = max(cx - reach(sx, wall[0][0]), 0), x1 = min(cx + reach(sx, wall[0][1]), g.dim[0] - 1);
                    const int c  = row ? g.dim[0] * (y + g.dim[1] * z) : 0;
                    const int b = cell_start[c + (row ? x0 : 0)], e = cell_start[c + (row ? x1 + 1 : 0)];
                    const float remp = rad_p * rad_p - ey * ey - ez * ez;
                    const bool prow  = row && rad_p > 0.f && remp >= 0.f;
                    const float sxp  = sqrtf(fmaxf(remp, 0.f));
                    const int x0p = max(cx - reach(sxp, wall[0][0]), x0), x1p = min(cx + reach(sxp, wall[0][1]), x1);
                    const int bp = cell_start[c + (prow ? x0p : 0)], ep = cell_start[c + (prow ? x1p + 1 : 0)];
                    rb[i] = row ? b : 0, re[i] = row ? e : 0;
                    pb[i] = prow ? bp : re[i], pe[i] = prow ? ep : re[i];
                }
#pragma unroll
                for (int i = 0; i <= 2 * RB; ++i) scan_range(rb[i], pb[i]), scan_range(pe[i], re[i]);
            }
            if (ball && best.dist(K - 1) <= rad * rad * 0.9999f) settled = true;
            else rad += g.cs;
        }
        if (settled) return;
    }
    if (!TIGHT) {
        scan_block3();
        if (best.dist(K - 1) < g.cs * g.cs * 0.9999f) return;
        r_first = 2;
    }
    for (int r = r_first; r < rmax; ++r) {
        const int z0 = max(cz - r, 0), z1 = min(cz + r, g.dim[2] - 1);
        const int y0 = max(cy - r, 0), y1 = min(cy + r, g.dim[1] - 1);
        const int x0 = max(cx - r, 0), x1 = min(cx + r, g.dim[0] - 1);
        for (int z = z0; z <= z1; ++z)
            for (int y = y0; y <= y1; ++y) {
                const bool face = (abs(z - cz) == r) || (abs(y - cy) == r);
                const int xstep = face ? 1 : max(x1 - x0, 1);
                for (int x = x0; x <= x1; x += xstep) {
                    if (!face && abs(x - cx) != r) continue;
                    const int c   = x + g.dim[0] * (y + g.dim[1] * z);
                    const int beg = cell_start[c], end = cell_start[c + 1];
                    for (int j = beg; j < end; ++j) {
                        const float4 n = sorted[j];
                        best.push(dist2(q, n.x, n.y, n.z), __float_as_int(n.w));
                    }
                }
            }
        const float bound = TIGHT ? fmaxf((float)r + margin - 1e-3f, 0.f) * g.cs : (float)r * g.cs;
        if (best.dist(K - 1) < bound * bound * 0.9999f) break;
    }
}

__device__ __forceinline__ unsigned long long wave_min_u64(unsigned long long v) {
#pragma unroll
    for (int o = 32; o > 0; o >>= 1) {
        const unsigned long long t = __shfl_xor(v, o, 64);
        v                          = t < v ? t : v;
    }
    return v;
}

template <int K>
__global__ __launch_bounds__(256) void knn_wave_kernel(const float* __restrict__ node_pos,
                                                       const float* __restrict__ node_w, int D,
                                                       const float* __restrict__ query, int n_query, int k,
                                                       int32_t* __restrict__ idx, float* __restrict__ weights,
                                                       KnnGridView grid) {
    const int v    = blockIdx.x * 4 + (threadIdx.x >> 6);
    const int lane = threadIdx.x & 63;
    if (v >= n_query) return;
    const KnnGridDesc g = *grid.desc;
    const f3 q = mk3(query[3 * (size_t)v], query[3 * (size_t)v + 1], query[3 * (size_t)v + 2]);
    KnnList<K> best;
    best.init();
    int cx, cy, cz;
    cell_of(g, q, cx, cy, cz);
    const int rmax = max(g.dim[0], max(g.dim[1], g.dim[2]));
    for (int r = 0; r < rmax; ++r) {
        const int side = 2 * r + 1, ncell = side * side * side;
        for (int c = lane; c < ncell; c += 64) {
            const int dx = c % side - r, dy = (c / side) % side - r, dz = c / (side * side) - r;
            if (max(abs(dx), max(abs(dy), abs(dz))) != r) continue;
            const int x = cx + dx, y = cy + dy, z = cz + dz;
            if (x < 0 || y < 0 || z < 0 || x >= g.dim[0] || y >= g.dim[1] || z >= g.dim[2]) continue;
            const int cell = x + g.dim[0] * (y + g.dim[1] * z);
            const int beg = grid.cell_start[cell], end = grid.cell_start[cell + 1];
            for (int j = beg; j < end; ++j) {
                const float4 n = grid.sorted[j];
                best.push(dist2(q, n.x, n.y, n.z), __float_as_int(n.w));
            }
        }
        const float bound = (float)r * g.cs, b2 = bound * bound * 0.9999f;
        int inside = 0;
#pragma unroll
        for (int j = 0; j < K; ++j) inside += best.dist(j) < b2 ? 1 : 0;
#pragma unroll
        for (int o = 32; o > 0; o >>= 1) inside += __shfl_xor(inside, o, 64);
        if (inside >= K) break;
    }
    int pos = 0;
    for (int j = 0; j < K; ++j) {
        unsigned long long key = KnnList<K>::EMPTY;
#pragma unroll
        for (int t = 0; t < K; ++t)
            if (t == pos) key = best.key[t];
        const int hi = (int)(unsigned int)key;
        const unsigned long long win = wave_min_u64(key);
        if (key == win && hi != 0x7fffffff) ++pos;
        if (lane == 0 && j < k) {
            const int n            = (int)(win & 0xffffffffu);
            const int node         = n == 0x7fffffff ? -1 : n;
            idx[(size_t)v * k + j] = node;
            if (weights) {
                float w = 0.f;
                if (node >= 0)
                    w = transformation_weight(mk3(node_pos[3 * node], node_pos[3 * node + 1], node_pos[3 * node + 2]),
                                              node_w[node], q);
                weights[(size_t)v * k + j] = w;
            }
        }
    }
}

template <int K, bool GRID>
__global__ __launch_bounds__(256) void knn_kernel(const float* __restrict__ node_pos,
                                                  const float* __restrict__ node_w, int D,
                                                  const float* __restrict__ query, int n_query, int k,
                                                  int32_t* __restrict__ idx, float* __restrict__ weights,
                                                  KnnGridView grid) {
    __shared__ float4 tile[GRID ? 1 : KNN_TILE];
    const int v       = blockIdx.x * blockDim.x + threadIdx.x;
    const bool active = v < n_query;
    f3 q              = mk3(0.f, 0.f, 0.f);
    if (active) q = mk3(query[3 * (size_t)v], query[3 * (size_t)v + 1], query[3 * (size_t)v + 2]);
    KnnList<K> best;
    if (GRID) {
        if (!active) return;
        knn_grid_query<K>(*grid.desc, grid.cell_start, grid.sorted, q, best);
    } else {
        knn_scan<K>(node_pos, D, q, best, tile);
        if (!active) return;
    }
    int out_i[K];
    float out_w[K];
#pragma unroll
    for (int j = 0; j < K; ++j) {
        out_i[j] = -1, out_w[j] = 0.f;
        if (j < k) {
            const int n = best.index(j);
            out_i[j]    = n;
            if (weights && n >= 0)
                out_w[j] = transformation_weight(mk3(node_pos[3 * n], node_pos[3 * n + 1], node_pos[3 * n + 2]), node_w[n], q);
        }
    }
    if (k == K && K % 4 == 0 && ((reinterpret_cast<uintptr_t>(idx) | reinterpret_cast<uintptr_t>(weights)) & 15u) == 0) {
#pragma unroll
        for (int h = 0; h < K / 4; ++h) {
            reinterpret_cast<int4*>(idx + (size_t)v * K)[h] = make_int4(out_i[4 * h], out_i[4 * h + 1], out_i[4 * h + 2], out_i[4 * h + 3]);
            if (weights)
                reinterpret_cast<float4*>(weights + (size_t)v * K)[h] = make_float4(out_w[4 * h], out_w[4 * h + 1], out_w[4 * h + 2], out_w[4 * h + 3]);
        }
        return;
    }
#pragma unroll
    for (int j = 0; j < K; ++j)
        if (j < k) {
            idx[(size_t)v * k + j] = out_i[j];
            if (weights) weights[(size_t)v * k + j] = out_w[j];
        }
}

template <int K>
__device__ __forceinline__ DQ calc_dqb(const KnnList<K>& nb, int k, const float* __restrict__ node_pos,
                                       const float* __restrict__ node_dq, const float* __restrict__ node_w, f3 p) {
    DQ sum = dq_identity();
    constexpr int G = K < 4 ? K : 4;
#pragma unroll
    for (int h = 0; h < K; h += G) {
        f3 g[G];
        float r[G];
        DQ q[G];
        bool on[G];
#pragma unroll
        for (int jj = 0; jj < G; ++jj) {
            const int j = h + jj;
            on[jj]      = j < k && nb.index(j) >= 0;
            const int n = on[jj] ? nb.index(j) : 0;
            g[jj] = mk3(node_pos[3 * n], node_pos[3 * n + 1], node_pos[3 * n + 2]), r[jj] = node_w[n];
            q[jj] = dq_load(node_dq + 8 * (size_t)n);
        }
#pragma unroll
        for (int jj = 0; jj < G; ++jj)
            if (on[jj]) sum = dq_mul(sum, dq_scale(q[jj], transformation_weight(g[jj], r[jj], p)));
    }
    return dq_normalize(sum);
}

template <int K, bool GRID>
__global__ __launch_bounds__(256) void warp_to_live_kernel(const float* __restrict__ node_pos,
                                                           const float* __restrict__ node_dq,
                                                           const float* __restrict__ node_w, int D, int k,
                                                           const float* __restrict__ verts,
                                                           const float* __restrict__ normals, int N,
                                                           float* __restrict__ out_verts,
                                                           float* __restrict__ out_normals, KnnGridView grid) {
    __shared__ float4 tile[GRID ? 1 : KNN_TILE];
    const int v       = blockIdx.x * blockDim.x + threadIdx.x;
    const bool active = v < N;
    f3 p              = mk3(0.f, 0.f, 0.f);
    if (active) p = mk3(verts[3 * (size_t)v], verts[3 * (size_t)v + 1], verts[3 * (size_t)v + 2]);
    KnnList<K> best;
    if (GRID) {
        if (!active) return;
        knn_grid_query<K>(*grid.desc, grid.cell_start, grid.sorted, p, best);
    } else {
        knn_scan<K>(node_pos, D, p, best, tile);
        if (!active) return;
    }
    const DQ dq = calc_dqb<K>(best, k, node_pos, node_dq, node_w, p);
    const f3 o  = dq_transform(dq, p);
    out_verts[3 * (size_t)v] = o.x, out_verts[3 * (size_t)v + 1] = o.y, out_verts[3 * (size_t)v + 2] = o.z;
    if (normals && out_normals) {
        const f3 nn = dq_transform(dq, mk3(normals[3 * (size_t)v], normals[3 * (size_t)v + 1],
                                           normals[3 * (size_t)v + 2]));
        out_normals[3 * (size_t)v] = nn.x, out_normals[3 * (size_t)v + 1] = nn.y,
                                out_normals[3 * (size_t)v + 2] = nn.z;
    }
}

template <int K>
__global__ __launch_bounds__(256) void warp_graph_kernel(const float* __restrict__ node_pos,
                                                         const float* __restrict__ node_dq,
                                                         const float* __restrict__ node_w, int k,
                                                         const int32_t* __restrict__ idx, const float* __restrict__ verts,
                                                         const float* __restrict__ normals, int N,
                                                         float* __restrict__ out_verts, float* __restrict__ out_normals) {
    const int v = blockIdx.x * blockDim.x + threadIdx.x;
    if (v >= N) return;
    KnnList<K> nb;
    nb.init();
    if (k == K && K % 4 == 0 && (reinterpret_cast<uintptr_t>(idx) & 15u) == 0) {
#pragma unroll
        for (int h = 0; h < K / 4; ++h) {
            const int4 n4 = reinterpret_cast<const int4*>(idx + (size_t)v * K)[h];
            nb.set_index(4 * h, n4.x), nb.set_index(4 * h + 1, n4.y), nb.set_index(4 * h + 2, n4.z), nb.set_index(4 * h + 3, n4.w);
        }
    } else {
#pragma unroll
        for (int j = 0; j < K; ++j)
            if (j < k) {
                const int n = idx[(size_t)v * k + j];
                nb.set_index(j, n);
            }
    }
    const f3 p  = mk3(verts[3 * (size_t)v], verts[3 * (size_t)v + 1], verts[3 * (size_t)v + 2]);
    const DQ dq = calc_dqb<K>(nb, k, node_pos, node_dq, node_w, p);
    const f3 o  = dq_transform(dq, p);
    out_verts[3 * (size_t)v] = o.x, out_verts[3 * (size_t)v + 1] = o.y, out_verts[3 * (size_t)v + 2] = o.z;
    if (normals && out_normals) {
        const f3 nn = dq_transform(dq, mk3(normals[3 * (size_t)v], normals[3 * (size_t)v + 1], normals[3 * (size_t)v + 2]));
        out_normals[3 * (size_t)v] = nn.x, out_normals[3 * (size_t)v + 1] = nn.y, out_normals[3 * (size_t)v + 2] = nn.z;
    }
}

template <bool GRID>
__global__ __launch_bounds__(256) void correspond_kernel(const float* __restrict__ canon_v,
                                                         const float* __restrict__ canon_n, int n_canon,
                                                         const float* __restrict__ live_v, int n_live,
                                                         float* __restrict__ out_v, float* __restrict__ out_n,
                                                         int32_t* __restrict__ out_idx, KnnGridView grid, bool rescan) {
    __shared__ float4 tile[GRID ? 1 : KNN_TILE];
    const int v       = blockIdx.x * blockDim.x + threadIdx.x;
    const bool active = v < n_live;
    f3 q              = mk3(0.f, 0.f, 0.f);
    if (active) q = mk3(live_v[3 * (size_t)v], live_v[3 * (size_t)v + 1], live_v[3 * (size_t)v + 2]);
    KnnList<1> best;
    if (GRID) {
        if (!active) return;
        knn_grid_query<1, true>(*grid.desc, grid.cell_start, grid.sorted, q, best, rescan);
    } else {
        knn_scan<1>(canon_v, n_canon, q, best, tile);
        if (!active) return;
    }
    const int n = best.index(0);
    if (out_idx) out_idx[v] = n;
    const size_t src = 3 * (size_t)max(n, 0), dst = 3 * (size_t)v;
    if (out_v) out_v[dst] = canon_v[src], out_v[dst + 1] = canon_v[src + 1], out_v[dst + 2] = canon_v[src + 2];
    if (out_n && canon_n)
        out_n[dst] = canon_n[src], out_n[dst + 1] = canon_n[src + 1], out_n[dst + 2] = canon_n[src + 2];
}

template <int K, bool GRID, bool FLAGS_ONLY>
__global__ __launch_bounds__(256) void dqb_support_kernel(const float* __restrict__ node_pos,
                                                          const float* __restrict__ node_dq,
                                                          const float* __restrict__ node_w, int D, int k,
                                                          const float* __restrict__ pts, int n,
                                                          float* __restrict__ out_dq, uint8_t* __restrict__ out_flag,
                                                          KnnGridView grid) {
    __shared__ float4 tile[GRID ? 1 : KNN_TILE];
    const int v       = blockIdx.x * blockDim.x + threadIdx.x;
    const bool active = v < n;
    f3 p              = mk3(0.f, 0.f, 0.f);
    if (active) p = mk3(pts[3 * (size_t)v], pts[3 * (size_t)v + 1], pts[3 * (size_t)v + 2]);
    auto quotient = [&](int m) __attribute__((always_inline)) {
        const double dx = (double)(p.x - node_pos[3 * m]), dy = (double)(p.y - node_pos[3 * m + 1]),
                     dz = (double)(p.z - node_pos[3 * m + 2]);
        return (float)sqrt(dx * dx + dy * dy + dz * dz) / node_w[m];
// ... 206 lines not shown
```

Before: 1597 frames/s.

## Fuse KNN queries into solver graph-row construction when the grid path applies

Adds a fused path in set_problem that builds the solver's row records directly from grid-based KNN searches, instead of running two separate KNN launches and then solve_build_graph. The shared KNN device code moves into a new header so the solver can call it. The aim is fewer kernel launches and no round trip through the ridx/rw/reg_idx arrays in global memory during problem setup. The fused path runs only when the grid is wanted and a capacity check passes; otherwise the old path is used.

```diff
diff --git a/dynfu_amd/csrc/capi.cpp b/dynfu_amd/csrc/capi.cpp
--- a/dynfu_amd/csrc/capi.cpp
+++ b/dynfu_amd/csrc/capi.cpp
@@ -162,6 +162,7 @@
     dfa::TeamPcg team;
     bool deterministic = false;
     bool just_reset = false;
+    bool graph_rows = false;
     long long* iters_total = nullptr;
     dfa_overlap_fn overlap_fn = nullptr;
     void* overlap_user        = nullptr;
@@ -975,13 +976,18 @@
     v.canon = canon_vertices, v.live = live_vertices;
     hipStream_t st = S(stream);
     const dfa::KnnGridView* grid = nullptr;
-    if (want_grid(D, (long)N + D)) {
+    if (want_grid(D, (long)N + D) || dfa::dev_env_int("DFA_GRAPH_GRID", 0) != 0) {
         HIP_TRY(dfa::knn_grid_build(s->grid.v, node_pos, D, st));
         grid = &s->grid.v;
     }
-    if (N > 0) HIP_TRY(dfa::launch_knn(node_pos, node_w, D, canon_vertices, N, s->k, v.ridx, v.rw, grid, st));
-    HIP_TRY(dfa::launch_knn(node_pos, node_w, D, node_pos, D, s->k, v.reg_idx, nullptr, grid, st));
-    HIP_TRY(dfa::solve_build_graph(v, s->state, s->ticket, 64, st));
+    s->graph_rows = grid && dfa::solve_graph_rows_fits(v);
+    if (s->graph_rows) {
+        HIP_TRY(dfa::solve_build_graph_rows(v, *grid, s->state, s->ticket, 64, st));
+    } else {
+        if (N > 0) HIP_TRY(dfa::launch_knn(node_pos, node_w, D, canon_vertices, N, s->k, v.ridx, v.rw, grid, st));
+        HIP_TRY(dfa::launch_knn(node_pos, node_w, D, node_pos, D, s->k, v.reg_idx, nullptr, grid, st));
+        HIP_TRY(dfa::solve_build_graph(v, s->state, s->ticket, 64, st));
+    }
     s->has_problem = true;
     s->just_reset  = true;
     return DFA_OK;
@@ -1506,6 +1512,15 @@
 
 }
 
+#ifdef DFA_DEV_AB
+extern "C" __attribute__((visibility("default"))) int dfa_dev_solver_graph_ptrs(dfa_solver* s, void** out) {
+    const dfa::SolveView& v = s->v;
+    void* p[] = {v.ridx, v.rw, v.rb, v.re, v.reg_idx, v.node_ptr, v.node_list, v.t, s->state, s->ticket, (void*)sizeof(dfa::SolveState)};
+    for (size_t i = 0; i < sizeof(p) / sizeof(p[0]); ++i) out[i] = p[i];
+    return s->graph_rows ? 1 : 0;
+}
+#endif
+
 #ifdef DFA_S6_DEBUG
 extern "C" __attribute__((visibility("default"))) int dfa_dev_solver6_ptrs(dfa_solver6* s, void** out) {
     const dfa::Solve6View& v = s->v;
diff --git a/dynfu_amd/csrc/knn_device.hpp b/dynfu_amd/csrc/knn_device.hpp
--- /dev/null
+++ b/dynfu_amd/csrc/knn_device.hpp
@@ -0,0 +1,275 @@
+#pragma once
+#include <hip/hip_runtime.h>
+
+#include "device_math.hpp"
+#include "dq_device.hpp"
+#include "kernels.hpp"
+
+namespace dfa {
+
+template <int K>
+struct KnnList {
+    unsigned long long key[K];
+    static constexpr unsigned long long EMPTY = 0x7f8000007fffffffull;
+    __device__ __forceinline__ static unsigned long long pack(float dist, int idx) {
+        return ((unsigned long long)__float_as_uint(dist) << 32) | (unsigned int)idx;
+    }
+    __device__ __forceinline__ void init() {
+#pragma unroll
+        for (int j = 0; j < K; ++j) key[j] = EMPTY;
+    }
+    __device__ __forceinline__ void push(float dist, int idx) {
+        const unsigned long long x = pack(dist, idx);
+        if (x < key[K - 1]) {
+            key[K - 1] = x;
+#pragma unroll
+            for (int j = K - 1; j > 0; --j) {
+                const unsigned long long a = key[j - 1], b = key[j];
+                key[j - 1] = a < b ? a : b, key[j] = a < b ? b : a;
+            }
+        }
+    }
+    __device__ __forceinline__ float dist(int j) const { return __uint_as_float((unsigned int)(key[j] >> 32)); }
+    __device__ __forceinline__ int raw_index(int j) const { return (int)(unsigned int)key[j]; }
+    __device__ __forceinline__ int index(int j) const { return raw_index(j) == 0x7fffffff ? -1 : raw_index(j); }
+    __device__ __forceinline__ void set_index(int j, int n) { key[j] = pack(__builtin_inff(), n < 0 ? 0x7fffffff : n); }
+};
+
+__device__ __forceinline__ float dist2(f3 q, float gx, float gy, float gz) {
+    const float d0 = q.x - gx, d1 = q.y - gy, d2 = q.z - gz;
+    return (d0 * d0 + d1 * d1) + d2 * d2;
+}
+
+template <int K>
+__device__ __forceinline__ void knn_ids_weights(const KnnList<K>& best, int k, const float* __restrict__ node_pos,
+                                                const float* __restrict__ node_w, bool with_weights, f3 q,
+                                                int (&out_i)[K], float (&out_w)[K]) {
+#pragma unroll
+    for (int j = 0; j < K; ++j) {
+        out_i[j] = -1, out_w[j] = 0.f;
+        if (j < k) {
+            const int n = best.index(j);
+            out_i[j]    = n;
+            if (with_weights && n >= 0)
+                out_w[j] = transformation_weight(mk3(node_pos[3 * n], node_pos[3 * n + 1], node_pos[3 * n + 2]), node_w[n], q);
+        }
+    }
+}
+
+__device__ __forceinline__ void cell_of(const KnnGridDesc& g, f3 p, int& cx, int& cy, int& cz) {
+    cx = min(max((int)floorf((p.x - g.bmin[0]) * g.inv_cs), 0), g.dim[0] - 1);
+    cy = min(max((int)floorf((p.y - g.bmin[1]) * g.inv_cs), 0), g.dim[1] - 1);
+    cz = min(max((int)floorf((p.z - g.bmin[2]) * g.inv_cs), 0), g.dim[2] - 1);
+}
+
+template <int K, bool TIGHT = false>
+__device__ __forceinline__ void knn_grid_query(const KnnGridDesc& g, const int32_t* __restrict__ cell_start,
+                                               const float4* __restrict__ sorted, f3 q, KnnList<K>& best, bool rescan = false) {
+    static_assert(!TIGHT || K == 1, "the tight stop bound re-scans the own cell: 1-NN only");
+    best.init();
+    int cx, cy, cz;
+    cell_of(g, q, cx, cy, cz);
+    float margin = 0.f;
+    float wall[3][2] = {{0.f, 0.f}, {0.f, 0.f}, {0.f, 0.f}};
+    bool inside      = false;
+    if (TIGHT) {
+        const float ux = (q.x - g.bmin[0]) * g.inv_cs - (float)cx, uy = (q.y - g.bmin[1]) * g.inv_cs - (float)cy,
+                    uz = (q.z - g.bmin[2]) * g.inv_cs - (float)cz;
+        const float m = fminf(fminf(fminf(ux, 1.f - ux), fminf(uy, 1.f - uy)), fminf(uz, 1.f - uz));
+        margin        = m > 0.f ? m : 0.f;
+        inside        = m >= 0.f;
+        const float u[3] = {ux, uy, uz};
+#pragma unroll
+        for (int c = 0; c < 3; ++c) wall[c][0] = fmaxf(u[c] - 1e-3f, 0.f) * g.cs, wall[c][1] = fmaxf(1.f - u[c] - 1e-3f, 0.f) * g.cs;
+    }
+    const int rmax = max(g.dim[0], max(g.dim[1], g.dim[2]));
+    int r_first    = 0;
+    auto scan_range = [&](int beg, int end) __attribute__((always_inline)) {
+        constexpr int KNN_BATCH = 4;
+        for (int j = beg; j < end; j += KNN_BATCH) {
+            float4 n[KNN_BATCH];
+#pragma unroll
+            for (int t = 0; t < KNN_BATCH; ++t) n[t] = sorted[min(j + t, end - 1)];
+#pragma unroll
+            for (int t = 0; t < KNN_BATCH; ++t)
+                if (j + t < end) best.push(dist2(q, n[t].x, n[t].y, n[t].z), __float_as_int(n[t].w));
+        }
+    };
+    auto scan_block3 = [&]() __attribute__((always_inline)) {
+        const int x0 = max(cx - 1, 0), x1 = min(cx + 1, g.dim[0] - 1);
+        int rbeg[9], rend[9];
+#pragma unroll
+        for (int i = 0; i < 9; ++i) {
+            const int z = cz - 1 + i / 3, y = cy - 1 + i % 3;
+            const bool in = z >= 0 && z < g.dim[2] && y >= 0 && y < g.dim[1];
+            const int c   = in ? g.dim[0] * (y + g.dim[1] * z) : 0;
+            const int b = cell_start[c + x0], e = cell_start[c + x1 + 1];
+            rbeg[i] = in ? b : 0, rend[i] = in ? e : 0;
+        }
+        constexpr int order[9] = {4, 1, 3, 5, 7, 0, 2, 6, 8};
+#pragma unroll
+        for (int i = 0; i < 9; ++i) scan_range(rbeg[order[i]], rend[order[i]]);
+    };
+    if (TIGHT) {
+        const int c0 = cx + g.dim[0] * (cy + g.dim[1] * cz);
+        scan_range(cell_start[c0], cell_start[c0 + 1]);
+        const float b0 = fmaxf(margin - 1e-3f, 0.f) * g.cs;
+        if (best.dist(K - 1) < b0 * b0 * 0.9999f) return;
+        {
+            const float d0 = best.dist(K - 1);
+            int rbeg[9], rend[9];
+#pragma unroll
+            for (int i = 0; i < 9; ++i) {
+                const int dz = i / 3 - 1, dy = i % 3 - 1, z = cz + dz, y = cy + dy;
+                const float ey = dy < 0 ? wall[1][0] : dy > 0 ? wall[1][1] : 0.f, ez = dz < 0 ? wall[2][0] : dz > 0 ? wall[2][1] : 0.f;
+                const float rb2 = ey * ey + ez * ez;
+                const bool keep = !inside || !(d0 < rb2 * 0.9999f);
+                const bool xl   = keep && (!inside || !(d0 < (rb2 + wall[0][0] * wall[0][0]) * 0.9999f));
+                const bool xr   = keep && (!inside || !(d0 < (rb2 + wall[0][1] * wall[0][1]) * 0.9999f));
+                const bool own  = dy == 0 && dz == 0;
+                const bool mid  = keep && (!own || (xl && xr));
+                const bool in   = z >= 0 && z < g.dim[2] && y >= 0 && y < g.dim[1] && (xl || xr || mid);
+                const int x0 = max(xl ? cx - 1 : (mid ? cx : cx + 1), 0), x1 = min(xr ? cx + 1 : (mid ? cx : cx - 1), g.dim[0] - 1);
+                const int c  = in ? g.dim[0] * (y + g.dim[1] * z) : 0;
+                const bool some = in && x0 <= x1;
+                const int b = cell_start[c + (some ? x0 : 0)], e = cell_start[c + (some ? x1 + 1 : 0)];
+                rbeg[i] = some ? b : 0, rend[i] = some ? e : 0;
+            }
+#pragma unroll
+            for (int i = 0; i < 9; ++i) scan_range(rbeg[i], rend[i]);
+        }
+        const float b1 = fmaxf(1.f + margin - 1e-3f, 0.f) * g.cs;
+        if (best.dist(K - 1) < b1 * b1 * 0.9999f) return;
+        r_first = 2;
+        constexpr int RB = 4;
+        auto reach = [&](float r, float w) { return r > w ? (int)fminf((r - w) * g.inv_cs, 1e6f) + 1 : 0; };
+        float rad   = best.dist(K - 1) < 3.0e38f ? sqrtf(best.dist(K - 1)) * 1.0001f : 2.f * g.cs;
+        bool settled = false;
+        for (int attempt = 0; attempt < RB; ++attempt) {
+            const float rad_p = attempt > 0 && !rescan ? rad - g.cs : -1.f;
+            const int nzl = reach(rad, wall[2][0]), nzh = reach(rad, wall[2][1]), nyl = reach(rad, wall[1][0]), nyh = reach(rad, wall[1][1]);
+            const bool ball = inside && !settled && max(max(nzl, nzh), max(nyl, nyh)) <= RB &&
+                              max(reach(rad, wall[0][0]), reach(rad, wall[0][1])) <= RB;
+            if (__ballot(ball) == 0ull) break;
+            int zl = 0, zh = 0;
+#pragma unroll
+            for (int v = 1; v <= RB; ++v) {
+                if (__ballot(ball && nzl >= v) != 0ull) zl = v;
+                if (__ballot(ball && nzh >= v) != 0ull) zh = v;
+            }
+            for (int sz = 0; sz <= 2 * max(zl, zh); ++sz) {
+                const int dz = (sz & 1) ? (sz + 1) / 2 : -(sz / 2);
+                if (dz > zh || -dz > zl) continue;
+                const float ez = dz == 0 ? 0.f : (dz < 0 ? wall[2][0] : wall[2][1]) + (float)(abs(dz) - 1) * g.cs;
+                int rb[2 * RB + 1], re[2 * RB + 1], pb[2 * RB + 1], pe[2 * RB + 1];
+#pragma unroll
+                for (int i = 0; i <= 2 * RB; ++i) {
+                    const int dy   = i - RB;
+                    const float ey = dy == 0 ? 0.f : (dy < 0 ? wall[1][0] : wall[1][1]) + (float)(abs(dy) - 1) * g.cs;
+                    const float rem = rad * rad - ey * ey - ez * ez;
+                    const int z = cz + dz, y = cy + dy;
+                    const bool row = ball && rem >= 0.f && dz <= nzh && -dz <= nzl && dy <= nyh && -dy <= nyl && z >= 0 &&
+                                     z < g.dim[2] && y >= 0 && y < g.dim[1];
+                    const float sx = sqrtf(fmaxf(rem, 0.f));
+                    const int x0 = max(cx - reach(sx, wall[0][0]), 0), x1 = min(cx + reach(sx, wall[0][1]), g.dim[0] - 1);
+                    const int c  = row ? g.dim[0] * (y + g.dim[1] * z) : 0;
+                    const int b = cell_start[c + (row ? x0 : 0)], e = cell_start[c + (row ? x1 + 1 : 0)];
+                    const float remp = rad_p * rad_p - ey * ey - ez * ez;
+                    const bool prow  = row && rad_p > 0.f && remp >= 0.f;
+                    const float sxp  = sqrtf(fmaxf(remp, 0.f));
+                    const int x0p = max(cx - reach(sxp, wall[0][0]), x0), x1p = min(cx + reach(sxp, wall[0][1]), x1);
+                    const int bp = cell_start[c + (prow ? x0p : 0)], ep = cell_start[c + (prow ? x1p + 1 : 0)];
+                    rb[i] = row ? b : 0, re[i] = row ? e : 0;
+                    pb[i] = prow ? bp : re[i], pe[i] = prow ? ep : re[i];
+                }
+#pragma unroll
+                for (int i = 0; i <= 2 * RB; ++i) scan_range(rb[i], pb[i]), scan_range(pe[i], re[i]);
+            }
+            if (ball && best.dist(K - 1) <= rad * rad * 0.9999f) settled = true;
+            else rad += g.cs;
+        }
+        if (settled) return;
+    }
+    if (!TIGHT) {
+        scan_block3();
+        if (best.dist(K - 1) < g.cs * g.cs * 0.9999f) return;
+        r_first = 2;
+    }
+    for (int r = r_first; r < rmax; ++r) {
+        const int z0 = max(cz - r, 0), z1 = min(cz + r, g.dim[2] - 1);
+        const int y0 = max(cy - r, 0), y1 = min(cy + r, g.dim[1] - 1);
+        const int x0 = max(cx - r, 0), x1 = min(cx + r, g.dim[0] - 1);
+        for (int z = z0; z <= z1; ++z)
+            for (int y = y0; y <= y1; ++y) {
+                const bool face = (abs(z - cz) == r) || (abs(y - cy) == r);
+                const int xstep = face ? 1 : max(x1 - x0, 1);
+                for (int x = x0; x <= x1; x += xstep) {
+                    if (!face && abs(x - cx) != r) continue;
+                    const int c   = x + g.dim[0] * (y + g.dim[1] * z);
+                    const int beg = cell_start[c], end = cell_start[c + 1];
+                    for (int j = beg; j < end; ++j) {
+                        const float4 n = sorted[j];
+                        best.push(dist2(q, n.x, n.y, n.z), __float_as_int(n.w));
+                    }
+                }
+            }
+        const float bound = TIGHT ? fmaxf((float)r + margin - 1e-3f, 0.f) * g.cs : (float)r * g.cs;
+        if (best.dist(K - 1) < bound * bound * 0.9999f) break;
+    }
+}
+
+__device__ __forceinline__ unsigned long long wave_min_u64(unsigned long long v) {
+#pragma unroll
+    for (int o = 32; o > 0; o >>= 1) {
+        const unsigned long long t = __shfl_xor(v, o, 64);
+        v                          = t < v ? t : v;
+    }
+    return v;
+}
+
+template <int K>
+__device__ __forceinline__ void knn_wave_search(const KnnGridDesc& g, const int32_t* __restrict__ cell_start,
+                                                const float4* __restrict__ sorted, f3 q, int lane, int (&out)[K]) {
+    KnnList<K> best;
+    best.init();
+    int cx, cy, cz;
+    cell_of(g, q, cx, cy, cz);
+    const int rmax = max(g.dim[0], max(g.dim[1], g.dim[2]));
+    for (int r = 0; r < rmax; ++r) {
+        const int side = 2 * r + 1, ncell = side * side * side;
+        for (int c = lane; c < ncell; c += 64) {
+            const int dx = c % side - r, dy = (c / side) % side - r, dz = c / (side * side) - r;
+            if (max(abs(dx), max(abs(dy), abs(dz))) != r) continue;
+            const int x = cx + dx, y = cy + dy, z = cz + dz;
+            if (x < 0 || y < 0 || z < 0 || x >= g.dim[0] || y >= g.dim[1] || z >= g.dim[2]) continue;
+            const int cell = x + g.dim[0] * (y + g.dim[1] * z);
+            const int beg = cell_start[cell], end = cell_start[cell + 1];
+            for (int j = beg; j < end; ++j) {
+                const float4 n = sorted[j];
+                best.push(dist2(q, n.x, n.y, n.z), __float_as_int(n.w));
+            }
+        }
+        const float bound = (float)r * g.cs, b2 = bound * bound * 0.9999f;
+        int inside = 0;
+#pragma unroll
+        for (int j = 0; j < K; ++j) inside += best.dist(j) < b2 ? 1 : 0;
+#pragma unroll
+        for (int o = 32; o > 0; o >>= 1) inside += __shfl_xor(inside, o, 64);
+        if (inside >= K) break;
+    }
+    int pos = 0;
+#pragma unroll
+    for (int j = 0; j < K; ++j) {
+        unsigned long long key = KnnList<K>::EMPTY;
+#pragma unroll
+        for (int t = 0; t < K; ++t)
+            if (t == pos) key = best.key[t];
+        const int hi = (int)(unsigned int)key;
+        const unsigned long long win = wave_min_u64(key);
+        if (key == win && hi != 0x7fffffff) ++pos;
+        const int n = (int)(win & 0xffffffffu);
+        out[j]      = n == 0x7fffffff ? -1 : n;
+    }
+}
+
+}
diff --git a/dynfu_amd/csrc/solve.hip b/dynfu_amd/csrc/solve.hip
--- a/dynfu_amd/csrc/solve.hip
+++ b/dynfu_amd/csrc/solve.hip
@@ -10,6 +10,7 @@
 #include "dq_device.hpp"
 #include "dev_switch.hpp"
 #include "kernels.hpp"
+#include "knn_device.hpp"
 #include "pcg_rules.hpp"
 #include "solve.hpp"
 
@@ -301,6 +302,61 @@
 }
 
 template <int K>
+__device__ __forceinline__ void store_record_head(const SolveView& s, size_t r, const int (&ids)[K], const float (&ws)[K], bool wide) {
+    const int k = s.k;
+    float* rec = s.re + r * (size_t)solve_rec_words(k);
+    if (wide) {
+        float4* rec4 = reinterpret_cast<float4*>(rec);
+        if (solve_rec_ids16(k)) {
+            uint32_t pk[K / 2];
+#pragma unroll
+            for (int j = 0; j < K / 2; ++j) {
+                const uint32_t lo = ids[2 * j] < 0 ? 0xffffu : (uint32_t)ids[2 * j], hi = ids[2 * j + 1] < 0 ? 0xffffu : (uint32_t)ids[2 * j + 1];
+                pk[j]             = (lo & 0xffffu) | (hi << 16);
+            }
+#pragma unroll
+            for (int q = 0; q < K / 8; ++q)
+                rec4[q] = make_float4(__uint_as_float(pk[4 * q]), __uint_as_float(pk[4 * q + 1]), __uint_as_float(pk[4 * q + 2]), __uint_as_float(pk[4 * q + 3]));
+#pragma unroll
+            for (int q = 0; q < K / 4; ++q) rec4[K / 8 + q] = make_float4(ws[4 * q], ws[4 * q + 1], ws[4 * q + 2], ws[4 * q + 3]);
+        } else {
+#pragma unroll
+            for (int q = 0; q < K / 4; ++q)
+                rec4[q] = make_float4(__int_as_float(ids[4 * q]), __int_as_float(ids[4 * q + 1]), __int_as_float(ids[4 * q + 2]), __int_as_float(ids[4 * q + 3]));
+#pragma unroll
+            for (int q = 0; q < K / 4; ++q) rec4[K / 4 + q] = make_float4(ws[4 * q], ws[4 * q + 1], ws[4 * q + 2], ws[4 * q + 3]);
+        }
+        return;
+    }
+    if (solve_rec_ids16(k)) {
+        uint16_t* h = reinterpret_cast<uint16_t*>(rec);
+#pragma unroll
+        for (int j = 0; j < K; ++j)
+            if (j < k) h[j] = ids[j] < 0 ? (uint16_t)0xffffu : (uint16_t)ids[j], rec[k / 2 + j] = ws[j];
+        return;
+    }
+#pragma unroll
+    for (int j = 0; j < K; ++j)
+        if (j < k) rec[j] = __int_as_float(ids[j]), rec[k + j] = ws[j];
+}
+
+template <int K>
+__device__ __forceinline__ void reg_row_slots(int m, int n, int (&ids)[K], float (&ws)[K]) {
+#pragma unroll
+    for (int j = 0; j < K; ++j) ids[j] = -1, ws[j] = 0.f;
+    if (m >= 0 && m != n) ids[0] = m, ws[0] = -1.f, ids[1] = n, ws[1] = +1.f;
+}
+
+template <int K>
+__device__ __forceinline__ void store_row_graph(const SolveView& s, size_t r, const int (&ids)[K], const float (&ws)[K]) {
+#pragma unroll
+    for (int q = 0; q < K / 4; ++q) {
+        reinterpret_cast<int4*>(s.ridx + r * K)[q]  = make_int4(ids[4 * q], ids[4 * q + 1], ids[4 * q + 2], ids[4 * q + 3]);
+        reinterpret_cast<float4*>(s.rw + r * K)[q] = make_float4(ws[4 * q], ws[4 * q + 1], ws[4 * q + 2], ws[4 * q + 3]);
+    }
+}
+
+template <int K>
 __global__ __launch_bounds__(256) void prepare_rows_kernel(SolveView s, SolveState* __restrict__ st,
                                                            unsigned int* __restrict__ ticket, int nticket) {
     const size_t R = (size_t)s.N + (size_t)s.D * s.k;
@@ -327,56 +383,63 @@
         }
     } else {
         const int e = (int)(r - (size_t)s.N), n = e / k, m = s.reg_idx[e];
-#pragma unroll
-        for (int j = 0; j < K; ++j) ids[j] = -1, ws[j] = 0.f;
-        if (m >= 0 && m != n) ids[0] = m, ws[0] = -1.f, ids[1] = n, ws[1] = +1.f;
-        if (wide) {
-#pragma unroll
-            for (int q = 0; q < K / 4; ++q) {
-                reinterpret_cast<int4*>(s.ridx + r * K)[q]  = make_int4(ids[4 * q], ids[4 * q + 1], ids[4 * q + 2], ids[4 * q + 3]);
-                reinterpret_cast<float4*>(s.rw + r * K)[q] = make_float4(ws[4 * q], ws[4 * q + 1], ws[4 * q + 2], ws[4 * q + 3]);
-            }
-        } else {
+        reg_row_slots<K>(m, n, ids, ws);
+        if (wide) store_row_graph<K>(s, r, ids, ws);
+        else {
 #pragma unroll
             for (int j = 0; j < K; ++j)
                 if (j < k) s.ridx[r * k + j] = ids[j], s.rw[r * k + j] = ws[j];
         }
         s.rb[3 * r + 0] = s.rb[3 * r + 1] = s.rb[3 * r + 2] = 0.f;
     }
-    float* rec = s.re + r * (size_t)solve_rec_words(k);
-    if (wide) {
-        float4* rec4 = reinterpret_cast<float4*>(rec);
-        if (solve_rec_ids16(k)) {
-            uint32_t pk[K / 2];
-#pragma unroll
-            for (int j = 0; j < K / 2; ++j) {
-                const uint32_t lo = ids[2 * j] < 0 ? 0xffffu : (uint32_t)ids[2 * j], hi = ids[2 * j + 1] < 0 ? 0xffffu : (uint32_t)ids[2 * j + 1];
-                pk[j]             = (lo & 0xffffu) | (hi << 16);
-            }
-#pragma unroll
-            for (int q = 0; q < K / 8; ++q)
-                rec4[q] = make_float4(__uint_as_float(pk[4 * q]), __uint_as_float(pk[4 * q + 1]), __uint_as_float(pk[4 * q + 2]), __uint_as_float(pk[4 * q + 3]));
-#pragma unroll
-            for (int q = 0; q < K / 4; ++q) rec4[K / 8 + q] = make_float4(ws[4 * q], ws[4 * q + 1], ws[4 * q + 2], ws[4 * q + 3]);
-        } else {
-#pragma unroll
-            for (int q = 0; q < K / 4; ++q)
-                rec4[q] = make_float4(__int_as_float(ids[4 * q]), __int_as_float(ids[4 * q + 1]), __int_as_float(ids[4 * q + 2]), __int_as_float(ids[4 * q + 3]));
-#pragma unroll
-            for (int q = 0; q < K / 4; ++q) rec4[K / 4 + q] = make_float4(ws[4 * q], ws[4 * q + 1], ws[4 * q + 2], ws[4 * q + 3]);
-        }
+    store_record_head<K>(s, r, ids, ws, wide);
+}
+
+template <int K>
+__global__ __launch_bounds__(256) void graph_rows_kernel(SolveView s, KnnGridView grid, SolveState* __restrict__ st,
+                                                         unsigned int* __restrict__ ticket, int nticket, int data_blocks) {
+    static_assert(K % 4 == 0, "rows by 16-byte stores");
+    if ((int)blockIdx.x < data_blocks) {
+        const int v = blockIdx.x * blockDim.x + threadIdx.x;
+        if (v >= s.N) return;
+        const f3 q = mk3(s.canon[3 * (size_t)v], s.canon[3 * (size_t)v + 1], s.canon[3 * (size_t)v + 2]);
+        KnnList<K> best;
+        knn_grid_query<K>(*grid.desc, grid.cell_start, grid.sorted, q, best);
+        int ids[K];
+        float ws[K];
+        knn_ids_weights<K>(best, K, s.node_pos, s.node_w, true, q, ids, ws);
+        const size_t r = (size_t)v;
+        store_row_graph<K>(s, r, ids, ws);
+        s.rb[3 * r + 0] = s.live[3 * r + 0] - q.x, s.rb[3 * r + 1] = s.live[3 * r + 1] - q.y, s.rb[3 * r + 2] = s.live[3 * r + 2] - q.z;
+        store_record_head<K>(s, r, ids, ws, true);
         return;
     }
-    if (solve_rec_ids16(k)) {
-        uint16_t* h = reinterpret_cast<uint16_t*>(rec);
-#pragma unroll
-        for (int j = 0; j < K; ++j)
-            if (j < k) h[j] = ids[j] < 0 ? (uint16_t)0xffffu : (uint16_t)ids[j], rec[k / 2 + j] = ws[j];
-        return;
-    }
+    const int b = (int)blockIdx.x - data_blocks;
+    const int i = b * (int)blockDim.x + (int)threadIdx.x;
+    if (i < 3 * s.D) s.t[i] = 0.f;
+    if (b == 0) {
+        unsigned int* w = (unsigned int*)st;
+        for (int j = threadIdx.x; j < (int)(sizeof(SolveState) / 4); j += blockDim.x) w[j] = 0u;
+        for (int j = threadIdx.x; j < nticket; j += blockDim.x) ticket[j] = 0u;
+    }
+    const int n = b * 4 + (int)(threadIdx.x >> 6), lane = threadIdx.x & 63;
+    if (n >= s.D) return;
+    const f3 q = mk3(s.node_pos[3 * (size_t)n], s.node_pos[3 * (size_t)n + 1], s.node_pos[3 * (size_t)n + 2]);
+    int near[K];
+    knn_wave_search<K>(*grid.desc, grid.cell_start, grid.sorted, q, lane, near);
+    if (lane >= K) return;
+    int m = -1;
 #pragma unroll
     for (int j = 0; j < K; ++j)
-        if (j < k) rec[j] = __int_as_float(ids[j]), rec[k + j] = ws[j];
+        if (j == lane) m = near[j];
+    const size_t e = (size_t)n * K + lane, r = (size_t)s.N + e;
+    s.reg_idx[e] = m;
+    int ids[K];
+    float ws[K];
+    reg_row_slots<K>(m, n, ids, ws);
+    store_row_graph<K>(s, r, ids, ws);
+    s.rb[3 * r + 0] = s.rb[3 * r + 1] = s.rb[3 * r + 2] = 0.f;
+    store_record_head<K>(s, r, ids, ws, true);
 }
 
 
@@ -1365,17 +1428,37 @@
     return hipGetLastError();
 }
 
-hipError_t solve_build_graph(const SolveView& s, SolveState* state, unsigned int* ticket, int nticket, hipStream_t st) {
-    const int D = s.D, N = s.N, k = s.k;
-    const size_t R = (size_t)N + (size_t)D * k, total = R * k;
-    const size_t threads = R > (size_t)3 * D ? R : (size_t)3 * D;
-    KDISPATCH(prepare_rows_kernel, k, <<<(unsigned)((threads + 255) / 256), 256, 0, st>>>(s, state, ticket, nticket));
+static hipError_t transpose_rows(const SolveView& s, hipStream_t st) {
+    const int D = s.D, k = s.k;
+    const size_t total = ((size_t)s.N + (size_t)D * k) * k;
     const size_t lds = sizeof(int32_t) * (size_t)D;
     tg_count_kernel<<<TG_BLOCKS, 1024, lds, st>>>(s.ridx, total, D, s.blk_hist);
     tg_colscan_kernel<<<(D + 255) / 256, 256, 0, st>>>(s.blk_hist, D);
     tg_fill_kernel<<<TG_BLOCKS, 1024, lds, st>>>(s.ridx, total, D, s.blk_hist, s.node_ptr, s.node_list);
     if (s.deterministic) sort_node_lists_kernel<<<D, 256, 0, st>>>(s.node_ptr, s.node_list);
     return hipGetLastError();
+}
+
+hipError_t solve_build_graph(const SolveView& s, SolveState* state, unsigned int* ticket, int nticket, hipStream_t st) {
+    const int D = s.D, N = s.N, k = s.k;
+    const size_t R = (size_t)N + (size_t)D * k;
+    const size_t threads = R > (size_t)3 * D ? R : (size_t)3 * D;
+    KDISPATCH(prepare_rows_kernel, k, <<<(unsigned)((threads + 255) / 256), 256, 0, st>>>(s, state, ticket, nticket));
+    return transpose_rows(s, st);
+}
+
+bool solve_graph_rows_fits(const SolveView& s) {
+    const int k = s.k;
+    return s.N > 0 && (k == 4 || k == 8 || k == 16) &&
+           ((reinterpret_cast<uintptr_t>(s.ridx) | reinterpret_cast<uintptr_t>(s.rw) | reinterpret_cast<uintptr_t>(s.re)) & 15u) == 0 &&
+           dev_env_int("DFA_GRAPH_ROWS", 1) != 0;
+}
+
+hipError_t solve_build_graph_rows(const SolveView& s, const KnnGridView& grid, SolveState* state, unsigned int* ticket,
+                                  int nticket, hipStream_t st) {
+    const int data_blocks = (s.N + 255) / 256, reg_blocks = (s.D + 3) / 4;
+    KDISPATCH(graph_rows_kernel, s.k, <<<data_blocks + reg_blocks, 256, 0, st>>>(s, grid, state, ticket, nticket, data_blocks));
+    return transpose_rows(s, st);
 }
 
 int solve_residual_blocks(const SolveView& s) {
diff --git a/dynfu_amd/csrc/solve.hpp b/dynfu_amd/csrc/solve.hpp
--- a/dynfu_amd/csrc/solve.hpp
+++ b/dynfu_amd/csrc/solve.hpp
@@ -1,6 +1,8 @@
 #pragma once
 #include <hip/hip_runtime.h>
 #include <stdint.h>
+
+#include "kernels.hpp"
 
 namespace dfa {
 
@@ -87,6 +89,9 @@
 
 constexpr int SOLVE_TG_BLOCKS = 256;
 hipError_t solve_build_graph(const SolveView& s, SolveState* state, unsigned int* ticket, int nticket, hipStream_t st);
+bool solve_graph_rows_fits(const SolveView& s);
+hipError_t solve_build_graph_rows(const SolveView& s, const KnnGridView& grid, SolveState* state, unsigned int* ticket,
+                                  int nticket, hipStream_t st);
 hipError_t solve_transpose_graph(const int32_t* ridx, size_t total, int D, int32_t* blk_hist, int32_t* node_ptr,
                                  uint32_t* node_list, hipStream_t st);
 int solve_residual_blocks(const SolveView& s);
diff --git a/dynfu_amd/csrc/warp.hip b/dynfu_amd/csrc/warp.hip
--- a/dynfu_amd/csrc/warp.hip
+++ b/dynfu_amd/csrc/warp.hip
@@ -3,43 +3,11 @@
 #include "dq_device.hpp"
 #include "dev_switch.hpp"
 #include "kernels.hpp"
+#include "knn_device.hpp"
 
 namespace dfa {
 
 constexpr int KNN_TILE = 1024;
-
-template <int K>
-struct KnnList {
-    unsigned long long key[K];
-    static constexpr unsigned long long EMPTY = 0x7f8000007fffffffull;
-    __device__ __forceinline__ static unsigned long long pack(float dist, int idx) {
-        return ((unsigned long long)__float_as_uint(dist) << 32) | (unsigned int)idx;
-    }
-    __device__ __forceinline__ void init() {
-#pragma unroll
-        for (int j = 0; j < K; ++j) key[j] = EMPTY;
-    }
-    __device__ __forceinline__ void push(float dist, int idx) {
-        const unsigned long long x = pack(dist, idx);
-        if (x < key[K - 1]) {
-            key[K - 1] = x;
-#pragma unroll
-            for (int j = K - 1; j > 0; --j) {
-                const unsigned long long a = key[j - 1], b = key[j];
-                key[j - 1] = a < b ? a : b, key[j] = a < b ? b : a;
-            }
-        }
-    }
-    __device__ __forceinline__ float dist(int j) const { return __uint_as_float((unsigned int)(key[j] >> 32)); }
-    __device__ __forceinline__ int raw_index(int j) const { return (int)(unsigned int)key[j]; }
-    __device__ __forceinline__ int index(int j) const { return raw_index(j) == 0x7fffffff ? -1 : raw_index(j); }
-    __device__ __forceinline__ void set_index(int j, int n) { key[j] = pack(__builtin_inff(), n < 0 ? 0x7fffffff : n); }
-};
-
-__device__ __forceinline__ float dist2(f3 q, float gx, float gy, float gz) {
-    const float d0 = q.x - gx, d1 = q.y - gy, d2 = q.z - gz;
-    return (d0 * d0 + d1 * d1) + d2 * d2;
-}
 
 template <int K>
 __device__ __forceinline__ void knn_scan(const float* __restrict__ node_pos, int D, f3 q, KnnList<K>& best,
@@ -99,12 +67,6 @@
             desc->dim[c] = min(max(n, 1), KNN_GRID_MAX_DIM);
         }
     }
-}
-
-__device__ __forceinline__ void cell_of(const KnnGridDesc& g, f3 p, int& cx, int& cy, int& cz) {
-    cx = min(max((int)floorf((p.x - g.bmin[0]) * g.inv_cs), 0), g.dim[0] - 1);
-    cy = min(max((int)floorf((p.y - g.bmin[1]) * g.inv_cs), 0), g.dim[1] - 1);
-    cz = min(max((int)floorf((p.z - g.bmin[2]) * g.inv_cs), 0), g.dim[2] - 1);
 }
 
 __global__ __launch_bounds__(256) void grid_count_kernel(const float* __restrict__ node_pos, int D,
@@ -407,170 +369,6 @@
     }
 }
 
-template <int K, bool TIGHT = false>
-__device__ __forceinline__ void knn_grid_query(const KnnGridDesc& g, const int32_t* __restrict__ cell_start,
-                                               const float4* __restrict__ sorted, f3 q, KnnList<K>& best, bool rescan = false) {
-    static_assert(!TIGHT || K == 1, "the tight stop bound re-scans the own cell: 1-NN only");
-    best.init();
-    int cx, cy, cz;
-    cell_of(g, q, cx, cy, cz);
-    float margin = 0.f;
-    float wall[3][2] = {{0.f, 0.f}, {0.f, 0.f}, {0.f, 0.f}};
-    bool inside      = false;
-    if (TIGHT) {
-        const float ux = (q.x - g.bmin[0]) * g.inv_cs - (float)cx, uy = (q.y - g.bmin[1]) * g.inv_cs - (float)cy,
-                    uz = (q.z - g.bmin[2]) * g.inv_cs - (float)cz;
-        const float m = fminf(fminf(fminf(ux, 1.f - ux), fminf(uy, 1.f - uy)), fminf(uz, 1.f - uz));
-        margin        = m > 0.f ? m : 0.f;
-        inside        = m >= 0.f;
-        const float u[3] = {ux, uy, uz};
-#pragma unroll
-        for (int c = 0; c < 3; ++c) wall[c][0] = fmaxf(u[c] - 1e-3f, 0.f) * g.cs, wall[c][1] = fmaxf(1.f - u[c] - 1e-3f, 0.f) * g.cs;
-    }
-    const int rmax = max(g.dim[0], max(g.dim[1], g.dim[2]));
-    int r_first    = 0;
-    auto scan_range = [&](int beg, int end) __attribute__((always_inline)) {
-        constexpr int KNN_BATCH = 4;
-        for (int j = beg; j < end; j += KNN_BATCH) {
-            float4 n[KNN_BATCH];
-#pragma unroll
-            for (int t = 0; t < KNN_BATCH; ++t) n[t] = sorted[min(j + t, end - 1)];
-#pragma unroll
-            for (int t = 0; t < KNN_BATCH; ++t)
-                if (j + t < end) best.push(dist2(q, n[t].x, n[t].y, n[t].z), __float_as_int(n[t].w));
-        }
-    };
-    auto scan_block3 = [&]() __attribute__((always_inline)) {
-        const int x0 = max(cx - 1, 0), x1 = min(cx + 1, g.dim[0] - 1);
-        int rbeg[9], rend[9];
-#pragma unroll
-        for (int i = 0; i < 9; ++i) {
-            const int z = cz - 1 + i / 3, y = cy - 1 + i % 3;
-            const bool in = z >= 0 && z < g.dim[2] && y >= 0 && y < g.dim[1];
-            const int c   = in ? g.dim[0] * (y + g.dim[1] * z) : 0;
-            const int b = cell_start[c + x0], e = cell_start[c + x1 + 1];
-            rbeg[i] = in ? b : 0, rend[i] = in ? e : 0;
-        }
-        constexpr int order[9] = {4, 1, 3, 5, 7, 0, 2, 6, 8};
-#pragma unroll
-        for (int i = 0; i < 9; ++i) scan_range(rbeg[order[i]], rend[order[i]]);
-    };
-    if (TIGHT) {
-        const int c0 = cx + g.dim[0] * (cy + g.dim[1] * cz);
-        scan_range(cell_start[c0], cell_start[c0 + 1]);
-        const float b0 = fmaxf(margin - 1e-3f, 0.f) * g.cs;
-        if (best.dist(K - 1) < b0 * b0 * 0.9999f) return;
-        {
-            const float d0 = best.dist(K - 1);
-            int rbeg[9], rend[9];
-#pragma unroll
-            for (int i = 0; i < 9; ++i) {
-                const int dz = i / 3 - 1, dy = i % 3 - 1, z = cz + dz, y = cy + dy;
-                const float ey = dy < 0 ? wall[1][0] : dy > 0 ? wall[1][1] : 0.f, ez = dz < 0 ? wall[2][0] : dz > 0 ? wall[2][1] : 0.f;
-                const float rb2 = ey * ey + ez * ez;
-                const bool keep = !inside || !(d0 < rb2 * 0.9999f);
-                const bool xl   = keep && (!inside || !(d0 < (rb2 + wall[0][0] * wall[0][0]) * 0.9999f));
-                const bool xr   = keep && (!inside || !(d0 < (rb2 + wall[0][1] * wall[0][1]) * 0.9999f));
-                const bool own  = dy == 0 && dz == 0;
-                const bool mid  = keep && (!own || (xl && xr));
-                const bool in   = z >= 0 && z < g.dim[2] && y >= 0 && y < g.dim[1] && (xl || xr || mid);
-                const int x0 = max(xl ? cx - 1 : (mid ? cx : cx + 1), 0), x1 = min(xr ? cx + 1 : (mid ? cx : cx - 1), g.dim[0] - 1);
-                const int c  = in ? g.dim[0] * (y + g.dim[1] * z) : 0;
-                const bool some = in && x0 <= x1;
-                const int b = cell_start[c + (some ? x0 : 0)], e = cell_start[c + (some ? x1 + 1 : 0)];
-                rbeg[i] = some ? b : 0, rend[i] = some ? e : 0;
-            }
-#pragma unroll
-            for (int i = 0; i < 9; ++i) scan_range(rbeg[i], rend[i]);
-        }
-        const float b1 = fmaxf(1.f + margin - 1e-3f, 0.f) * g.cs;
-        if (best.dist(K - 1) < b1 * b1 * 0.9999f) return;
-        r_first = 2;
-        constexpr int RB = 4;
-        auto reach = [&](float r, float w) { return r > w ? (int)fminf((r - w) * g.inv_cs, 1e6f) + 1 : 0; };
-        float rad   = best.dist(K - 1) < 3.0e38f ? sqrtf(best.dist(K - 1)) * 1.0001f : 2.f * g.cs;
-        bool settled = false;
-        for (int attempt = 0; attempt < RB; ++attempt) {
-            const float rad_p = attempt > 0 && !rescan ? rad - g.cs : -1.f;
-            const int nzl = reach(rad, wall[2][0]), nzh = reach(rad, wall[2][1]), nyl = reach(rad, wall[1][0]), nyh = reach(rad, wall[1][1]);
-            const bool ball = inside && !settled && max(max(nzl, nzh), max(nyl, nyh)) <= RB &&
-                              max(reach(rad, wall[0][0]), reach(rad, wall[0][1])) <= RB;
-            if (__ballot(ball) == 0ull) break;
-            int zl = 0, zh = 0;
-#pragma unroll
-            for (int v = 1; v <= RB; ++v) {
-                if (__ballot(ball && nzl >= v) != 0ull) zl = v;
-                if (__ballot(ball && nzh >= v) != 0ull) zh = v;
-            }
-            for (int sz = 0; sz <= 2 * max(zl, zh); ++sz) {
-                const int dz = (sz & 1) ? (sz + 1) / 2 : -(sz / 2);
-                if (dz > zh || -dz > zl) continue;
-                const float ez = dz == 0 ? 0.f : (dz < 0 ? wall[2][0] : wall[2][1]) + (float)(abs(dz) - 1) * g.cs;
-                int rb[2 * RB + 1], re[2 * RB + 1], pb[2 * RB + 1], pe[2 * RB + 1];
-#pragma unroll
-                for (int i = 0; i <= 2 * RB; ++i) {
-                    const int dy   = i - RB;
-                    const float ey = dy == 0 ? 0.f : (dy < 0 ? wall[1][0] : wall[1][1]) + (float)(abs(dy) - 1) * g.cs;
-                    const float rem = rad * rad - ey * ey - ez * ez;
-                    const int z = cz + dz, y = cy + dy;
-                    const bool row = ball && rem >= 0.f && dz <= nzh && -dz <= nzl && dy <= nyh && -dy <= nyl && z >= 0 &&
-                                     z < g.dim[2] && y >= 0 && y < g.dim[1];
-                    const float sx = sqrtf(fmaxf(rem, 0.f));
-                    const int x0 = max(cx - reach(sx, wall[0][0]), 0), x1 = min(cx + reach(sx, wall[0][1]), g.dim[0] - 1);
-                    const int c  = row ? g.dim[0] * (y + g.dim[1] * z) : 0;
-                    const int b = cell_start[c + (row ? x0 : 0)], e = cell_start[c + (row ? x1 + 1 : 0)];
-                    const float remp = rad_p * rad_p - ey * ey - ez * ez;
-                    const bool prow  = row && rad_p > 0.f && remp >= 0.f;
-                    const float sxp  = sqrtf(fmaxf(remp, 0.f));
-                    const int x0p = max(cx - reach(sxp, wall[0][0]), x0), x1p = min(cx + reach(sxp, wall[0][1]), x1);
-                    const int bp = cell_start[c + (prow ? x0p : 0)], ep = cell_start[c + (prow ? x1p + 1 : 0)];
-                    rb[i] = row ? b : 0, re[i] = row ? e : 0;
-                    pb[i] = prow ? bp : re[i], pe[i] = prow ? ep : re[i];
-                }
-#pragma unroll
-                for (int i = 0; i <= 2 * RB; ++i) scan_range(rb[i], pb[i]), scan_range(pe[i], re[i]);
-            }
-            if (ball && best.dist(K - 1) <= rad * rad * 0.9999f) settled = true;
-            else rad += g.cs;
-        }
-        if (settled) return;
-    }
-    if (!TIGHT) {
-        scan_block3();
-        if (best.dist(K - 1) < g.cs * g.cs * 0.9999f) return;
-        r_first = 2;
-    }
-    for (int r = r_first; r < rmax; ++r) {
-        const int z0 = max(cz - r, 0), z1 = min(cz + r, g.dim[2] - 1);
-        const int y0 = max(cy - r, 0), y1 = min(cy + r, g.dim[1] - 1);
-        const int x0 = max(cx - r, 0), x1 = min(cx + r, g.dim[0] - 1);
-        for (int z = z0; z <= z1; ++z)
-            for (int y = y0; y <= y1; ++y) {
-                const bool face = (abs(z - cz) == r) || (abs(y - cy) == r);
-                const int xstep = face ? 1 : max(x1 - x0, 1);
-                for (int x = x0; x <= x1; x += xstep) {
-                    if (!face && abs(x - cx) != r) continue;
-                    const int c   = x + g.dim[0] * (y + g.dim[1] * z);
-                    const int beg = cell_start[c], end = cell_start[c + 1];
-                    for (int j = beg; j < end; ++j) {
-                        const float4 n = sorted[j];
-                        best.push(dist2(q, n.x, n.y, n.z), __float_as_int(n.w));
-                    }
-                }
-            }
-        const float bound = TIGHT ? fmaxf((float)r + margin - 1e-3f, 0.f) * g.cs : (float)r * g.cs;
-        if (best.dist(K - 1) < bound * bound * 0.9999f) break;
-    }
-}
-
-__device__ __forceinline__ unsigned long long wave_min_u64(unsigned long long v) {
-#pragma unroll
-    for (int o = 32; o > 0; o >>= 1) {
-        const unsigned long long t = __shfl_xor(v, o, 64);
-        v                          = t < v ? t : v;
-    }
-    return v;
-}
 
 template <int K>
 __global__ __launch_bounds__(256) void knn_wave_kernel(const float* __restrict__ node_pos,
@@ -583,45 +381,13 @@
     if (v >= n_query) return;
     const KnnGridDesc g = *grid.desc;
     const f3 q = mk3(query[3 * (size_t)v], query[3 * (size_t)v + 1], query[3 * (size_t)v + 2]);
-    KnnList<K> best;
-    best.init();
-    int cx, cy, cz;
-    cell_of(g, q, cx, cy, cz);
-    const int rmax = max(g.dim[0], max(g.dim[1], g.dim[2]));
-    for (int r = 0; r < rmax; ++r) {
-        const int side = 2 * r + 1, ncell = side * side * side;
-        for (int c = lane; c < ncell; c += 64) {
-            const int dx = c % side - r, dy = (c / side) % side - r, dz = c / (side * side) - r;
-            if (max(abs(dx), max(abs(dy), abs(dz))) != r) continue;
-            const int x = cx + dx, y = cy + dy, z = cz + dz;
-            if (x < 0 || y < 0 || z < 0 || x >= g.dim[0] || y >= g.dim[1] || z >= g.dim[2]) continue;
-            const int cell = x + g.dim[0] * (y + g.dim[1] * z);
-            const int beg = grid.cell_start[cell], end = grid.cell_start[cell + 1];
-            for (int j = beg; j < end; ++j) {
-                const float4 n = grid.sorted[j];
-                best.push(dist2(q, n.x, n.y, n.z), __float_as_int(n.w));
-            }
-        }
-        const float bound = (float)r * g.cs, b2 = bound * bound * 0.9999f;
-        int inside = 0;
-#pragma unroll
-        for (int j = 0; j < K; ++j) inside += best.dist(j) < b2 ? 1 : 0;
-#pragma unroll
-        for (int o = 32; o > 0; o >>= 1) inside += __shfl_xor(inside, o, 64);
-        if (inside >= K) break;
-    }
-    int pos = 0;
-    for (int j = 0; j < K; ++j) {
-        unsigned long long key = KnnList<K>::EMPTY;
-#pragma unroll
-        for (int t = 0; t < K; ++t)
-            if (t == pos) key = best.key[t];
-        const int hi = (int)(unsigned int)key;
-        const unsigned long long win = wave_min_u64(key);
-        if (key == win && hi != 0x7fffffff) ++pos;
-        if (lane == 0 && j < k) {
-            const int n            = (int)(win & 0xffffffffu);
-            const int node         = n == 0x7fffffff ? -1 : n;
+    int near[K];
+    knn_wave_search<K>(g, grid.cell_start, grid.sorted, q, lane, near);
+    if (lane != 0) return;
+#pragma unroll
+    for (int j = 0; j < K; ++j)
+        if (j < k) {
+            const int node         = near[j];
             idx[(size_t)v * k + j] = node;
             if (weights) {
                 float w = 0.f;
@@ -631,7 +397,6 @@
                 weights[(size_t)v * k + j] = w;
             }
         }
-    }
 }
 
 template <int K, bool GRID>
@@ -655,16 +420,7 @@
     }
     int out_i[K];
     float out_w[K];
-#pragma unroll
-    for (int j = 0; j < K; ++j) {
-        out_i[j] = -1, out_w[j] = 0.f;
-        if (j < k) {
-            const int n = best.index(j);
-            out_i[j]    = n;
-            if (weights && n >= 0)
-                out_w[j] = transformation_weight(mk3(node_pos[3 * n], node_pos[3 * n + 1], node_pos[3 * n + 2]), node_w[n], q);
-        }
-    }
+    knn_ids_weights<K>(best, k, node_pos, node_w, weights != nullptr, q, out_i, out_w);
     if (k == K && K % 4 == 0 && ((reinterpret_cast<uintptr_t>(idx) | reinterpret_cast<uintptr_t>(weights)) & 15u) == 0) {
 #pragma unroll
         for (int h = 0; h < K / 4; ++h) {
```

Result: faster. 1636 frames/s, median of 6 (+2.5%).
